# Dizzy-cell/HOUV

Measured on AMD Instinct MI355X. Metric: registration pairs/sec (2048-pt partial pairs), higher is better.
Workload: dtype f32; 1 GPU; HOUV solve_model, 2048x2048-pt pairs, batch 256/GPU, K=64 restarts x 200 Adam iterations + retry stages (BASELINE configs[1]); pairs_per_gpu=256, points=2048, kernel=64, iters=200, icp_refine=False, parallelism=dp1 (pair shards, one RCCL all-gather of [steps*P,12] per rank)

## Files before the change

houv_amd/_lib.py:

```python
import ctypes
import os

import torch

_HERE = os.path.dirname(os.path.abspath(__file__))
LIB_PATH = os.environ.get("HOUV_HIP_LIB") or os.path.join(_HERE, "lib", "libhouv_hip.so")
ABI_VERSION = 2

_c_f = ctypes.c_void_p
_int = ctypes.c_int
_dbl = ctypes.c_double
_flt = ctypes.c_float

_SIGNATURES = {
    "houv_abi_version": (ctypes.c_int, []),
    "houv_last_error": (ctypes.c_char_p, []),
    "houv_build_id": (ctypes.c_char_p, []),
    "houv_debug_set": (ctypes.c_int, [ctypes.c_char_p, ctypes.c_longlong]),
    "houv_chamfer_forward": (ctypes.c_int, [_c_f, _c_f, _int, _int, _int, _c_f, _c_f, _c_f, _c_f, _c_f]),
    "houv_chamfer_backward": (ctypes.c_int, [_c_f, _c_f, _int, _int, _int, _c_f, _c_f, _c_f, _c_f, _c_f, _c_f, _c_f]),
    "houv_kabsch": (ctypes.c_int, [_c_f, _c_f, _c_f, _int, _int, _c_f, _c_f, _c_f]),
    "houv_solve_iterate": (ctypes.c_int, [_c_f, _c_f, _int, _int, _int, _int, _c_f, _int, _int, _int, _int, _int, _int,
                                          _int, _int, _dbl, _dbl, _dbl, _dbl, _flt, _c_f, _c_f, _c_f, _c_f, _c_f, _c_f,
                                          _c_f]),
    "houv_solve_iterate_large": (ctypes.c_int, [_c_f, _c_f, _int, _int, _int, _int, _c_f, _int, _int, _int, _int, _int, _int,
                                                _int, _int, _dbl, _dbl, _dbl, _dbl, _flt, _c_f, _c_f, _c_f, _c_f, _c_f, _c_f,
                                                _c_f]),
    "houv_solve_iterate_pruned": (ctypes.c_int, [_c_f, _c_f, _int, _int, _int, _int, _c_f, _int, _int, _int, _int, _int,
                                                 _int, _int, _int, _dbl, _dbl, _dbl, _dbl, _flt, _c_f, _c_f, _c_f, _c_f,
                                                 _c_f, _c_f, _c_f, _int, _int, _c_f]),
    "houv_solve_variant": (ctypes.c_int, [_int, _int, _int, ctypes.POINTER(ctypes.c_int), ctypes.POINTER(ctypes.c_int),
                                          ctypes.POINTER(ctypes.c_int)]),
    "houv_solve_lds_bytes": (ctypes.c_longlong, [_int, _int, _int]),
    "houv_solve_walk_variant": (ctypes.c_int, [_int]),
    "houv_kd_sort": (ctypes.c_int, [_c_f, _int, _int, _int, _int, _c_f, _c_f, _c_f]),
    "houv_icp_refine": (ctypes.c_int, [_c_f, _c_f, _int, _int, _int, _c_f, _flt, _int, _flt, _flt, _c_f, _c_f, _c_f, _c_f, _c_f]),
    "houv_knn": (ctypes.c_int, [_c_f, _int, _int, _int, _c_f, _c_f]),
    "houv_edgeconv1": (ctypes.c_int, [_c_f, _c_f, _int, _int, _int, _c_f, _c_f, _c_f, _c_f, _c_f]),
    "houv_max_over_k": (ctypes.c_int, [_c_f, ctypes.c_longlong, _int, _int, _c_f, _int, _c_f]),
    "houv_gemm_f32": (ctypes.c_int, [_c_f, _c_f, _c_f, _int, _int, _int, _int, _int, _int, _int, _int, _int] +
                      [ctypes.c_longlong] * 6 + [_flt, _c_f, _c_f, _c_f, _int, ctypes.c_longlong, ctypes.c_longlong,
                                                 _int, _c_f]),
    "houv_attention_f32": (ctypes.c_int, [_c_f, _c_f, _c_f, _c_f, _int, _int, _int, _int, _int, _int, _int, _int, _int] +
                           [ctypes.c_longlong] * 4 + [_flt, _c_f]),
    "houv_layernorm": (ctypes.c_int, [_c_f, ctypes.c_longlong, _int, _c_f, _c_f, _flt, _c_f, _c_f, _c_f]),
    "houv_softmax_rows": (ctypes.c_int, [_c_f, ctypes.c_longlong, _int, _c_f]),
    "houv_softmax_corr": (ctypes.c_int, [_c_f, _int, _int, _int, _c_f, _c_f, _c_f]),
    "houv_furthest_point_sample": (ctypes.c_int, [_c_f, _int, _int, _int, _c_f, _c_f]),
    "houv_knn_cross": (ctypes.c_int, [_c_f, _c_f, _int, _int, _int, _int, _c_f, _c_f, _c_f]),
    "houv_gather_points": (ctypes.c_int, [_c_f, _c_f, _int, _int, _int, _int, _c_f, _c_f]),
    "houv_ball_query": (ctypes.c_int, [_c_f, _c_f, _int, _int, _int, _flt, _flt, _int, _c_f, _c_f, _c_f]),
    "houv_three_interpolate": (ctypes.c_int, [_c_f, _c_f, _c_f, _int, _int, _int, _int, _c_f, _c_f]),
    "houv_scatter_points_grad": (ctypes.c_int, [_c_f, _c_f, _c_f, _int, _int, _int, _int, _int, _c_f, _c_f, _c_f]),
    "houv_scatter_points_workspace_bytes": (ctypes.c_longlong, [_int, _int, _int]),
    "houv_emd_forward": (ctypes.c_int, [_c_f, _c_f, _int, _int, _int, _flt, _int, _c_f, _c_f, _c_f, _c_f, _c_f]),
    "houv_emd_workspace_bytes": (ctypes.c_longlong, [_int, _int]),
    "houv_emd_backward": (ctypes.c_int, [_c_f, _c_f, _int, _int, _c_f, _c_f, _c_f, _c_f]),
    "houv_rri_features": (ctypes.c_int, [_c_f, _c_f, _int, _int, _int, _int, _int, _c_f, _c_f]),
    "houv_gmm_params": (ctypes.c_int, [_c_f, _c_f, _int, _int, _int, _c_f, _c_f, _c_f, _c_f]),
    "houv_gmm_register": (ctypes.c_int, [_c_f, _c_f, _c_f, _c_f, _int, _int, _c_f, _c_f]),
    "houv_idam_simmat": (ctypes.c_int, [_c_f] * 4 + [_int] * 4 + [_c_f] * 15),
    "houv_edge_diff": (ctypes.c_int, [_c_f, _c_f, _int, _int, _int, _int, _int, _int, _c_f, _c_f]),
    "houv_mlp2_max": (ctypes.c_int, [_c_f, _int, _int, _int, _c_f, _int, _c_f, ctypes.c_longlong, _c_f, _c_f, _int, _c_f, _c_f, _c_f, _c_f]),
    "houv_mlp2_max_workspace_bytes": (ctypes.c_longlong, [_int, _int, _int]),
    "houv_mlp2_max_arg": (ctypes.c_int, [_c_f, _int, _int, _int, _c_f, _int, _c_f, ctypes.c_longlong, _c_f, _c_f, _int, _c_f, _c_f, _c_f, _c_f, _c_f]),
    "houv_mlp2_max_arg_workspace_bytes": (ctypes.c_longlong, [_int, _int, _int]),
    "houv_mlp2_max_backward": (ctypes.c_int, [_c_f, _int, _int, _int, _c_f, _int, _c_f, ctypes.c_longlong, _c_f, _int, _c_f, _c_f,
                                              _c_f, _c_f, _c_f, _int] + [_c_f] * 9),
    "houv_mlp2_max_backward_workspace_bytes": (ctypes.c_longlong, [_int] * 6),
    "houv_mlp2_max_backward_rows": (ctypes.c_int, [_int, _int, _int]),
    "houv_pcn_fold": (ctypes.c_int, [_c_f, _c_f, _c_f, _int, _int, _int, _c_f, _c_f, _c_f, _c_f, _c_f, _c_f, _c_f]),
    "houv_pcn_fold_backward": (ctypes.c_int, [_c_f, _c_f, _c_f, _int, _int, _int] + [_c_f] * 14 + [ctypes.c_longlong, _c_f]),
    "houv_pcn_fold_backward_workspace_bytes": (ctypes.c_longlong, [_int, _int, _int]),
    "houv_knn_feat": (ctypes.c_int, [_c_f, _int, _int, _int, _int, _int, _c_f, _c_f, _c_f]),
    "houv_dense_conv": (ctypes.c_int, [_c_f, _int, _c_f, _int, _int, _int, _int] + [_c_f] * 6 + [_int, _c_f, _int, _c_f]),
    "houv_dense_conv_arg": (ctypes.c_int, [_c_f, _int, _c_f, _int, _int, _int, _int] + [_c_f] * 6 + [_int, _c_f, _int, _c_f, _c_f]),
    "houv_dense_conv_backward": (ctypes.c_int, [_c_f, _int, _c_f, _int, _int, _int, _int] + [_c_f] * 6 +
                                 [_int, _c_f, _c_f, _int, _c_f, _int, _c_f, _int] + [_c_f] * 7 + [ctypes.c_longlong, _c_f]),
    "houv_dense_conv_backward_workspace_bytes": (ctypes.c_longlong, [_int, _int, _int, _int]),
    "houv_sa_attn": (ctypes.c_int, [_c_f, _int, _c_f, _int, _c_f, _int, _int, _int, _int] + [_c_f] * 5 + [_int, _c_f, _int, _c_f]),
    "houv_sa_attn_backward": (ctypes.c_int, [_c_f, _int, _c_f, _int, _int, _int, _int, _c_f, _c_f, _c_f, _c_f, _int, _c_f, _int, _c_f, _int,
                                             _c_f, _c_f, _c_f, _c_f, ctypes.c_longlong, _c_f]),
    "houv_sa_attn_backward_workspace_bytes": (ctypes.c_longlong, [_int, _int, _int, _int]),
    "houv_edge_pool": (ctypes.c_int, [_c_f, _int, _c_f, _c_f, _int, _int, _int, _int, _int, _c_f, _int, _c_f, _c_f]),
    "houv_edge_pool_backward": (ctypes.c_int, [_c_f, _int, _c_f, _c_f, _c_f, _int, _int, _int, _int, _int, _c_f, _int, _c_f,
                                               ctypes.c_longlong, _c_f]),
    "houv_edge_pool_backward_workspace_bytes": (ctypes.c_longlong, [_int, _int, _int, _int]),
    "houv_ef_expand": (ctypes.c_int, [_c_f, _int, _c_f, _int, _int, _int, _int, _int, _c_f, _int, _c_f, _c_f, _c_f, _int, _c_f, _c_f]),
    "houv_ef_expand_backward": (ctypes.c_int, [_c_f, _int, _c_f, _c_f, _int, _int, _int, _int, _int, _c_f, _int, _c_f, _c_f, _int, _c_f,
                                               _int, _c_f, _c_f, _c_f, _c_f, ctypes.c_longlong, _c_f]),
    "houv_ef_expand_backward_workspace_bytes": (ctypes.c_longlong, [_int] * 5),
    "houv_pose_forward": (ctypes.c_int,[_c_f, _int, _int, _int, _c_f, _int, _c_f, _c_f, _c_f, _c_f]),
}

_lib = None


class HouvHipError(RuntimeError):
    pass


def exported_symbols():
    return sorted(_SIGNATURES)


def load():
    global _lib
    if _lib is not None:
        return _lib
    if not os.path.exists(LIB_PATH):
        raise HouvHipError(
            f"{LIB_PATH} not found: build it with `python -c 'import __graft_entry__ as g; g.build()'` "
            "(or `make -C houv_amd/csrc`). houv_amd has no CPU fallback.")
    lib = ctypes.CDLL(LIB_PATH)
    for name, (res, args) in _SIGNATURES.items():
        fn = getattr(lib, name)
        fn.restype = res
        fn.argtypes = args
    if lib.houv_abi_version() != ABI_VERSION:
        raise HouvHipError(f"libhouv_hip.so ABI {lib.houv_abi_version()} != expected {ABI_VERSION}")
    _lib = lib
    return lib


def solve_variant(N, M, pruned=False, with_mode=False):
    b, q, m = ctypes.c_int(0), ctypes.c_int(0), ctypes.c_int(0)
    check(load().houv_solve_variant(int(N), int(M), int(bool(pruned)), ctypes.byref(b), ctypes.byref(q), ctypes.byref(m)),
          "houv_solve_variant")
    return (b.value, q.value, m.value) if with_mode else (b.value, q.value)


def solve_walk_variant(need):
    v = load().houv_solve_walk_variant(int(need))
    if v < 0:
        raise HouvHipError(f"houv_solve_walk_variant failed: {last_error()}")
    return v


def build_id():
    return load().houv_build_id().decode()


def debug_set(name, value):
    check(load().houv_debug_set(name.encode(), int(value)), "houv_debug_set")


def last_error():
    return load().houv_last_error().decode("utf-8", "replace")


def check(ok, what):
    if ok != 1:
        raise HouvHipError(f"{what} failed: {last_error()}")


def ptr(t):
    return None if t is None else ctypes.c_void_p(t.data_ptr())


def stream_of(t):
    return ctypes.c_void_p(torch.cuda.current_stream(t.device).cuda_stream)


def require_gpu(*tensors, dtype=None):
    for t in tensors:
        if t is None:
            continue
        if not t.is_cuda:
            raise HouvHipError("houv_amd ops run on an MI355X only: got a CPU tensor (there is no CPU fallback)")
        if not t.is_contiguous():
            raise HouvHipError("houv_amd ops need contiguous tensors")
    dev = [t.device for t in tensors if t is not None]
    if any(d != dev[0] for d in dev):
        raise HouvHipError("all tensors must live on the same device")


def require_gpu_any(*tensors):
    ts = [t for t in tensors if t is not None]
    for t in ts:
        if not t.is_cuda:
            raise HouvHipError("houv_amd ops run on an MI355X only: got a CPU tensor (there is no CPU fallback)")
        if t.dtype != torch.float32:
            raise HouvHipError(f"expected float32, got {t.dtype}")
    if any(t.device != ts[0].device for t in ts):
        raise HouvHipError("all tensors must live on the same device")
```

houv_amd/csrc/capi.hip:

```cpp
#include <stdarg.h>
#include <string.h>

#include "../../include/houv_hip.h"
#include "houv_common.h"

namespace houv {

static thread_local char g_err[512] = "";

void set_error(const char* fmt, ...) {
  va_list ap;
  va_start(ap, fmt);
  vsnprintf(g_err, sizeof(g_err), fmt, ap);
  va_end(ap);
  fprintf(stderr, "[houv_hip] %s\n", g_err);
}

DebugKnobs g_debug;

namespace {

__global__ void pose_kernel(const float* __restrict__ params, int n, int angle_base, int trans_mode,
                            float* __restrict__ R, float* __restrict__ T) {
  const int i = blockIdx.x * blockDim.x + threadIdx.x;
  if (i >= n) return;
  float p[8];
#pragma unroll
  for (int k = 0; k < 8; ++k) p[k] = params[i * 8 + k];
  Pose f;
  pose_forward(p, angle_base, trans_mode, f);
#pragma unroll
  for (int k = 0; k < 9; ++k) R[i * 9 + k] = f.R[k];
#pragma unroll
  for (int k = 0; k < 3; ++k) T[i * 3 + k] = f.T[k];
}

__global__ void move_kernel(const float* __restrict__ src, const float* __restrict__ R, const float* __restrict__ T,
                            size_t total, int N, float* __restrict__ moved) {
  for (size_t e = (size_t)blockIdx.x * blockDim.x + threadIdx.x; e < total; e += (size_t)gridDim.x * blockDim.x) {
    const size_t b = e / N;
    const float* r = R + b * 9;
    const float x = src[e * 3 + 0], y = src[e * 3 + 1], z = src[e * 3 + 2];
    moved[e * 3 + 0] = __builtin_fmaf(z, r[2], __builtin_fmaf(y, r[1], x * r[0])) + T[b * 3 + 0];
    moved[e * 3 + 1] = __builtin_fmaf(z, r[5], __builtin_fmaf(y, r[4], x * r[3])) + T[b * 3 + 1];
    moved[e * 3 + 2] = __builtin_fmaf(z, r[8], __builtin_fmaf(y, r[7], x * r[6])) + T[b * 3 + 2];
  }
}

}
}

extern "C" int houv_abi_version(void) { return HOUV_ABI_VERSION; }

extern "C" const char* houv_last_error(void) { return houv::g_err; }

extern "C" int houv_debug_set(const char* name, long long value) {
  using namespace houv;
  const struct { const char* name; std::atomic<int>* knob; long long lo, hi, step; } ints[] = {
      {"solve_predict", &g_debug.pred_mode, 0, 2, 1}, {"knn_split", &g_debug.knn_split, 0, 1, 1},
      {"attn_split", &g_debug.attn_split, 0, 1, 1},   {"gemm_split", &g_debug.gemm_split, 0, 6, 3}};
  if (name && !strcmp(name, "solve_stats")) {
    g_debug.stats = (unsigned long long)value;
    return 1;
  }
  if (name && !strcmp(name, "solve_walk_hist")) {
    g_debug.walk_hist = (unsigned long long)value;
    return 1;
  }
  if (name && !strcmp(name, "solve_cull_stats")) {
    g_debug.cull_stats = (unsigned long long)value;
    return 1;
  }
  for (const auto& k : ints)
    if (name && !strcmp(name, k.name) && value >= k.lo && value <= k.hi && value % k.step == 0) {
      *k.knob = (int)value;
      return 1;
    }
  set_error("houv_debug_set: unknown switch or value out of range: %s = %lld", name ? name : "(null)", value);
  return 0;
}

#ifndef HOUV_BUILD_ID
#define HOUV_BUILD_ID "unknown"
#endif
extern "C" const char* houv_build_id(void) { return HOUV_BUILD_ID; }

extern "C" int houv_pose_forward(const float* params, int n, int angle_base, int trans_mode, const float* src, int N,
                                 float* R, float* T, float* moved, void* stream) {
  using namespace houv;
  if (n < 0 || !params || !R || !T || angle_base < 0 || angle_base > 3 || trans_mode < 0 || trans_mode > 1) {
    set_error("houv_pose_forward: bad argument");
    return 0;
  }
  if (n == 0) return 1;
  hipStream_t s = (hipStream_t)stream;
  pose_kernel<<<(n + 255) / 256, 256, 0, s>>>(params, n, angle_base, trans_mode, R, T);
  if (src && moved && N > 0) {
    const size_t total = (size_t)n * N;
    size_t blocks = (total + 255) / 256;
    if (blocks > 16384) blocks = 16384;
    move_kernel<<<(unsigned)blocks, 256, 0, s>>>(src, R, T, total, N, moved);
  }
  return check_launch("houv_pose_forward") ? 1 : 0;
}
```

houv_amd/csrc/houv_common.h:

```cpp
#pragma once
#include <hip/hip_runtime.h>
#include <stdint.h>
#include <stdio.h>

#include <atomic>

#include "houv_math.h"

namespace houv {

constexpr int kWave = 64;
constexpr int kSub = 32;
constexpr int kTrk = 16;

void set_error(const char* fmt, ...);
struct SolveCommon;
__attribute__((visibility("hidden"))) int solve_check_args(const char* who, const SolveCommon& a, int use_views);
__attribute__((visibility("hidden"))) bool scatter_index_launch(const int* keys, int B, int N, int M, int* offsets, int* order,
                                                                hipStream_t stream);
inline bool check_launch(const char* what) {
  hipError_t e = hipGetLastError();
  if (e != hipSuccess) {
    set_error("%s: %s", what, hipGetErrorString(e));
    return false;
  }
  return true;
}

struct DebugKnobs {
  std::atomic<int> pred_mode{0};
  std::atomic<unsigned long long> stats{0ull};
  std::atomic<unsigned long long> walk_hist{0ull};
  std::atomic<unsigned long long> cull_stats{0ull};
  std::atomic<int> knn_split{1};
  std::atomic<int> attn_split{1};
  std::atomic<int> gemm_split{6};
};
extern DebugKnobs g_debug;

template <int MET>
__device__ __forceinline__ float metric_sqdist(float dx, float dy, float dz) {
  if constexpr (MET == 0) return __builtin_fmaf(dz, dz, __builtin_fmaf(dy, dy, dx * dx));
  else if constexpr (MET == 1) return __builtin_fmaf(dz, dz, dy * dy);
  else if constexpr (MET == 2) return __builtin_fmaf(dz, dz, dx * dx);
  else return __builtin_fmaf(dy, dy, dx * dx);
}

__device__ __forceinline__ float min3f(float a, float b, float c) {
  return __builtin_fminf(__builtin_fminf(a, b), c);
}

__device__ __forceinline__ float wave_sum(float v) {
#pragma unroll
  for (int o = 32; o > 0; o >>= 1) v += __shfl_xor(v, o, kWave);
  return v;
}

__device__ __forceinline__ int wave_sum_i(int v) {
#pragma unroll
  for (int o = 32; o > 0; o >>= 1) v += __shfl_xor(v, o, kWave);
  return v;
}

template <int CTRL, int ROW_MASK = 0xf, int BANK_MASK = 0xf>
__device__ __forceinline__ float dpp_f(float v) {
  return __int_as_float(__builtin_amdgcn_update_dpp(0, __float_as_int(v), CTRL, ROW_MASK, BANK_MASK, true));
}
template <int CTRL, int ROW_MASK = 0xf, int BANK_MASK = 0xf>
__device__ __forceinline__ int dpp_i(int v) {
  return __builtin_amdgcn_update_dpp(0, v, CTRL, ROW_MASK, BANK_MASK, true);
}

__device__ __forceinline__ float wave_sum_to_lane63(float v) {
  v += dpp_f<0x111>(v);
  v += dpp_f<0x112>(v);
  v += dpp_f<0x114>(v);
  v += dpp_f<0x118>(v);
  v += dpp_f<0x142, 0xa>(v);
  v += dpp_f<0x143, 0xc>(v);
  return v;
}

__device__ __forceinline__ int wave_max_to_lane63(int v) {
  v = max(v, dpp_i<0x111>(v));
  v = max(v, dpp_i<0x112>(v));
  v = max(v, dpp_i<0x114>(v));
  v = max(v, dpp_i<0x118>(v));
  v = max(v, dpp_i<0x142, 0xa>(v));
  v = max(v, dpp_i<0x143, 0xc>(v));
  return v;
}

template <int CTRL, int ROW_MASK = 0xf>
__device__ __forceinline__ float fmax_dpp(float v) {
  return __builtin_fmaxf(v, __int_as_float(__builtin_amdgcn_update_dpp(__float_as_int(v), __float_as_int(v), CTRL, ROW_MASK, 0xf, false)));
}
__device__ __forceinline__ float wave_fmax_to_lane63(float v) {
  v = fmax_dpp<0x111>(v);
  v = fmax_dpp<0x112>(v);
  v = fmax_dpp<0x114>(v);
  v = fmax_dpp<0x118>(v);
  v = fmax_dpp<0x142, 0xa>(v);
  v = fmax_dpp<0x143, 0xc>(v);
  return v;
}

__device__ __forceinline__ int wave_incl_scan_dpp(int x) {
  int v = x + dpp_i<0x111>(x);
  v += dpp_i<0x112>(x);
  v += dpp_i<0x113>(x);
  v += dpp_i<0x114, 0xf, 0xe>(v);
  v += dpp_i<0x118, 0xf, 0xc>(v);
  v += dpp_i<0x142, 0xa>(v);
  v += dpp_i<0x143, 0xc>(v);
  return v;
}

__device__ __forceinline__ int wave_incl_scan_i(int v) {
  const int lane = threadIdx.x & 63;
#pragma unroll
  for (int o = 1; o < 64; o <<= 1) {
    int n = __shfl_up(v, o, kWave);
    if (lane >= o) v += n;
  }
  return v;
}

}
```

houv_amd/csrc/houv_math.h:

```cpp
#pragma once
#include <math.h>

#if defined(__HIPCC__)
#define HOUV_HD __host__ __device__
#else
#define HOUV_HD
#endif

namespace houv {

constexpr float kPiF = 3.14159274101257324f;

enum TransMode { kTransHouv = 0, kTransSolve = 1 };

HOUV_HD inline float tsqrt(float x) { return sqrtf(x); }
HOUV_HD inline double tsqrt(double x) { return sqrt(x); }

struct Pose {
  float R[9];
  float T[3];
  float u[3], inv_vnorm, sin_t, cos_t, chat[3], inv_cnorm, sigma, a, s;
};

HOUV_HD inline void pose_forward(const float p[8], int angle_base, int trans_mode, Pose& o) {
// ... 90 lines not shown
  bool bad = false;
#pragma unroll
  for (int m = 0; m < 4; ++m) r.cd[m][0] = r.cd[m][1] = 0.f;
#pragma unroll
  for (int m = 0; m < NMET; ++m) {
    const float kk = (float)((m == 0) ? k_full : k_view);
    r.cd[m][0] = acc[(m * 2 + 0) * acc_stride] / kk;
    r.cd[m][1] = acc[(m * 2 + 1) * acc_stride] / kk;
    pick[m] = (r.cd[m][0] <= r.cd[m][1]) ? 0 : 1;
    val[m] = r.cd[m][pick[m]];
    if (r.cd[m][0] != r.cd[m][0] || r.cd[m][1] != r.cd[m][1]) { val[m] = NAN; bad = true; }
    const float w = ((m == 0) ? 6.0f : 1.0f) * loss_scale / kk;
    const float* ac = acc + (m * 2 + pick[m]) * acc_stride;
#pragma unroll
    for (int i = 0; i < 3; ++i) gT[i] += w * ac[1 + i];
#pragma unroll
    for (int i = 0; i < 9; ++i) Mm[i] += w * ac[4 + i];
  }
  r.score = val[0];
  r.loss = val[0] * 6.0f;
  if constexpr (NMET == 4) r.loss = r.loss + (val[1] + val[2] + val[3]);
  if (bad) {
#pragma unroll
    for (int i = 0; i < 3; ++i) gT[i] = NAN;
#pragma unroll
    for (int i = 0; i < 9; ++i) Mm[i] = NAN;
  }
  pose_backward(f, trans_mode, gT, Mm, r.g);
}

HOUV_HD inline void solve_tail_step(const float g[8], double* state, int f64_params, AdamScalars asc, double beta1, double beta2,
                                    double eps, int angle_base, int trans_mode, Pose& next) {
  if (f64_params) {
    for (int k = 0; k < 8; ++k)
      adam_step<double>(state[k], state[8 + k], state[16 + k], (double)g[k], asc, beta1, beta2, eps);
  } else {
    for (int k = 0; k < 8; ++k) {
      float pp = (float)state[k], mm = (float)state[8 + k], vv = (float)state[16 + k];
      adam_step<float>(pp, mm, vv, g[k], asc, beta1, beta2, eps);
      state[k] = pp; state[8 + k] = mm; state[16 + k] = vv;
    }
  }
  float p[8];
#pragma unroll
  for (int k = 0; k < 8; ++k) p[k] = (float)state[k];
  pose_forward(p, angle_base, trans_mode, next);
}

constexpr int kTermAnchorFloats = 20;
constexpr float kTermRel = 1e-3f;
constexpr float kTermAbs = 1e-6f;
constexpr float kTermMoveErr = 1e-6f;

template <int NMET>
HOUV_HD inline unsigned term_masks(const float* anchor, const float* R, const float* T, float radius) {
  float fr = 0.f, ft = 0.f, tn = 0.f, ta = 0.f;
#pragma unroll
  for (int i = 0; i < 9; ++i) {
    const float d = R[i] - anchor[8 + i];
    fr += d * d;
  }
#pragma unroll
  for (int i = 0; i < 3; ++i) {
    const float d = T[i] - anchor[17 + i];
    ft += d * d;
    tn += T[i] * T[i];
    ta += anchor[17 + i] * anchor[17 + i];
  }
  const float delta2 = 2.0f * (sqrtf(fr) * radius + sqrtf(ft));
  const float abs_margin = kTermAbs + kTermMoveErr * (2.0f * radius + sqrtf(tn) + sqrtf(ta));
  unsigned need = ((1u << NMET) - 1u) * 0x11u;
#pragma unroll
  for (int m = 0; m < NMET; ++m) {
    const float c0 = anchor[2 * m], c1 = anchor[2 * m + 1];
    const float slack = delta2 + kTermRel * (fabsf(c0) + fabsf(c1) + delta2) + abs_margin;
    const unsigned drop1 = (c0 + slack < c1) ? (0x10u << m) : 0u;
    const unsigned drop0 = (c1 + slack < c0) ? (1u << m) : 0u;
    need &= ~(drop0 | drop1);
  }
  return need;
}

constexpr float kTermDefectMax = 1e-3f;
constexpr float kTermDefectErr = 1e-6f;

HOUV_HD inline float term_rot_defect(const float* M) {
  float s = 0.f;
#pragma unroll
  for (int i = 0; i < 3; ++i)
#pragma unroll
    for (int j = i; j < 3; ++j) {
      const float g = M[i] * M[j] + M[3 + i] * M[3 + j] + M[6 + i] * M[6 + j] - ((i == j) ? 1.0f : 0.0f);
      s += ((i == j) ? 1.0f : 2.0f) * g * g;
    }
  return sqrtf(s) + kTermDefectErr;
}

HOUV_HD inline void term_travel(const float* Rz, const float* Tz, const float* R, const float* T, float def_now, float radius,
                                float& d, float& tz) {
  float fr = 0.f, ft = 0.f, ta = 0.f;
#pragma unroll
  for (int i = 0; i < 9; ++i) {
    const float e = R[i] - Rz[i];
    fr += e * e;
  }
#pragma unroll
  for (int i = 0; i < 3; ++i) {
    const float e = T[i] - Tz[i];
    ft += e * e;
    ta += Tz[i] * Tz[i];
  }
  const float fro = sqrtf(fr), defect = def_now + term_rot_defect(Rz);
  const float tight = fro * 0.70710683f + 2.0f * defect;
  const bool ok = (fr <= 2.0f) & (defect <= kTermDefectMax) & (tight < fro);
  d = (ok ? tight : fro) * radius + sqrtf(ft);
  tz = sqrtf(ta);
}

template <int NMET>
HOUV_HD inline unsigned term_anchor_masks(const float* cd, const float* fresh, const float* stale, int stride,
                                          unsigned stale_bits, const float* R, const float* T, float radius_in) {
  const float radius = fabsf(radius_in);
  const float def_now = term_rot_defect(R);
  const float tn = sqrtf(T[0] * T[0] + T[1] * T[1] + T[2] * T[2]);
  float d_f, t_f;
  term_travel(fresh, fresh + 9, R, T, def_now, radius, d_f, t_f);
  unsigned need = ((1u << NMET) - 1u) * 0x11u;
#pragma unroll
  for (int m = 0; m < NMET; ++m) {
    float Rs[9], Ts[3], d_s, t_s;
#pragma unroll
    for (int i = 0; i < 9; ++i) Rs[i] = stale[(m * 12 + i) * stride];
#pragma unroll
    for (int i = 0; i < 3; ++i) Ts[i] = stale[(m * 12 + 9 + i) * stride];
    term_travel(Rs, Ts, R, T, def_now, radius, d_s, t_s);
    const bool s0 = (stale_bits >> m) & 1u, s1 = (stale_bits >> (4 + m)) & 1u;
    const float d0 = s0 ? d_s : d_f, d1 = s1 ? d_s : d_f;
    const float t0 = s0 ? t_s : t_f, t1 = s1 ? t_s : t_f;
    const float c0 = cd[2 * m], c1 = cd[2 * m + 1];
    const float dd = d0 + d1;
    const float slack = dd + kTermRel * (fabsf(c0) + fabsf(c1) + dd) + kTermAbs +
                        kTermMoveErr * (2.0f * radius + tn + 0.5f * (t0 + t1));
    const unsigned drop1 = (c0 + slack < c1) ? (0x10u << m) : 0u;
    const unsigned drop0 = (c1 + slack < c0) ? (1u << m) : 0u;
    need &= ~(drop0 | drop1);
  }
  return need;
}

constexpr int kWalkSets[] = {6, 11, 12, 13, 15};
constexpr int kNumWalkSets = (int)(sizeof(kWalkSets) / sizeof(kWalkSets[0]));
constexpr int walk_step_cost(unsigned mset) {
  const int k0 = (int)(mset & 1u), k1 = (int)((mset >> 1) & 1u), k2 = (int)((mset >> 2) & 1u), k3 = (int)((mset >> 3) & 1u);
  return 16 * (2 * (k0 + k1 + k2 + ((k0 | k3) ? 1 : 0)) + 2 * k1 + (k0 + k1 + k2 + k3)) + 5 * (k0 + k1 + k2 + k3);
}
constexpr bool walk_instantiated(unsigned mset) {
  for (int i = 0; i < kNumWalkSets; ++i)
    if ((unsigned)kWalkSets[i] == mset) return true;
  return false;
}
constexpr unsigned walk_variant(unsigned need) {
  unsigned best = 15u;
  for (int i = 0; i < kNumWalkSets; ++i) {
    const unsigned s = (unsigned)kWalkSets[i];
    if ((s & need) == need && walk_step_cost(s) < walk_step_cost(best)) best = s;
  }
  return best;
}
static_assert(walk_instantiated(15u) && walk_variant(15u) == 15u && walk_step_cost(15u) == 16 * 14 + 20, "today's code is a variant");
constexpr unsigned long long walk_variant_table() {
  unsigned long long t = 0ull;
  for (unsigned n = 0; n < 16u; ++n) t |= (unsigned long long)walk_variant(n) << (4 * n);
  return t;
}

HOUV_HD inline float box_med3(float a, float b, float c) {
#if defined(__HIP_DEVICE_COMPILE__)
  return __builtin_amdgcn_fmed3f(a, b, c);
#else
  if (a != a || b != b || c != c) return fminf(fminf(a, b), c);
  return fmaxf(fminf(a, b), fminf(fmaxf(a, b), c));
#endif
}

template <int NMET>
HOUV_HD inline bool box_within_bounds(float dx, float dy, float dz, const float* b, unsigned mset) {
  if constexpr (NMET == 4) {
    const float xx = dx * dx, yy = dy * dy;
    const float s3 = __builtin_fmaf(dy, dy, xx), s1 = __builtin_fmaf(dz, dz, yy), s2 = __builtin_fmaf(dz, dz, xx);
    const float s0 = __builtin_fmaf(dz, dz, s3);
    bool in = false;
    if (mset & 1u) in |= s0 <= b[0];
    if (mset & 2u) in |= s1 <= b[1];
    if (mset & 4u) in |= s2 <= b[2];
    if (mset & 8u) in |= s3 <= b[3];
    return in;
  } else {
    return __builtin_fmaf(dz, dz, __builtin_fmaf(dy, dy, dx * dx)) <= b[0];
  }
}

template <int NMET>
HOUV_HD inline bool box_test_query(const float* q, const float* lo, const float* hi, const float* ub, unsigned mset) {
  return box_within_bounds<NMET>(q[0] - box_med3(q[0], lo[0], hi[0]), q[1] - box_med3(q[1], lo[1], hi[1]),
                                 q[2] - box_med3(q[2], lo[2], hi[2]), ub, mset);
}

HOUV_HD inline float box_group_gap(float glo, float ghi, float lo, float hi) {
  return fmaxf(fmaxf(fminf(lo, hi) - ghi, glo - fmaxf(lo, hi)), 0.0f);
}

template <int NMET>
HOUV_HD inline bool box_test_group(const float* glo, const float* ghi, const float* lo, const float* hi, const float* gub,
                                   unsigned mset) {
  return box_within_bounds<NMET>(box_group_gap(glo[0], ghi[0], lo[0], hi[0]), box_group_gap(glo[1], ghi[1], lo[1], hi[1]),
                                 box_group_gap(glo[2], ghi[2], lo[2], hi[2]), gub, mset);
}

template <typename T>
HOUV_HD inline void svd3x3(const T H[9], T U[9], T S[3], T V[9]) {
  T B[9];
  for (int i = 0; i < 9; ++i) { B[i] = H[i]; V[i] = (i % 4 == 0) ? (T)1 : (T)0; }
  const int P[3] = {0, 0, 1}, Qi[3] = {1, 2, 2};
  for (int sweep = 0; sweep < 12; ++sweep) {
    T off = 0;
    for (int r = 0; r < 3; ++r) {
      const int p = P[r], q = Qi[r];
      const T a = B[0 * 3 + p] * B[0 * 3 + p] + B[1 * 3 + p] * B[1 * 3 + p] + B[2 * 3 + p] * B[2 * 3 + p];
      const T b = B[0 * 3 + q] * B[0 * 3 + q] + B[1 * 3 + q] * B[1 * 3 + q] + B[2 * 3 + q] * B[2 * 3 + q];
      const T g = B[0 * 3 + p] * B[0 * 3 + q] + B[1 * 3 + p] * B[1 * 3 + q] + B[2 * 3 + p] * B[2 * 3 + q];
      const T eps2 = sizeof(T) == 4 ? (T)1e-14 : (T)1e-31;
      if (g * g <= eps2 * a * b) continue;
      off += (T)1;
      const T zeta = (b - a) / ((T)2 * g);
      const T az = zeta < 0 ? -zeta : zeta;
      const T t = (zeta < 0 ? (T)-1 : (T)1) / (az + tsqrt((T)1 + zeta * zeta));
      const T c = (T)1 / tsqrt((T)1 + t * t);
      const T s = c * t;
      for (int i = 0; i < 3; ++i) {
        const T bp = B[i * 3 + p], bq = B[i * 3 + q];
        B[i * 3 + p] = c * bp - s * bq;
        B[i * 3 + q] = s * bp + c * bq;
        const T vp = V[i * 3 + p], vq = V[i * 3 + q];
        V[i * 3 + p] = c * vp - s * vq;
        V[i * 3 + q] = s * vp + c * vq;
      }
    }
    if (off == (T)0) break;
  }
  for (int j = 0; j < 3; ++j)
    S[j] = tsqrt(B[0 * 3 + j] * B[0 * 3 + j] + B[1 * 3 + j] * B[1 * 3 + j] + B[2 * 3 + j] * B[2 * 3 + j]);
  auto swapcol = [&](int x, int y) {
    T ts = S[x]; S[x] = S[y]; S[y] = ts;
    for (int i = 0; i < 3; ++i) {
      T tb = B[i * 3 + x]; B[i * 3 + x] = B[i * 3 + y]; B[i * 3 + y] = tb;
      T tv = V[i * 3 + x]; V[i * 3 + x] = V[i * 3 + y]; V[i * 3 + y] = tv;
    }
  };
  if (S[0] < S[1]) swapcol(0, 1);
  if (S[1] < S[2]) swapcol(1, 2);
  if (S[0] < S[1]) swapcol(0, 1);
  const T tiny = S[0] * (sizeof(T) == 4 ? (T)1e-6 : (T)1e-13);
  for (int j = 0; j < 2; ++j) {
    if (S[j] > tiny && S[j] > (T)0) {
      for (int i = 0; i < 3; ++i) U[i * 3 + j] = B[i * 3 + j] / S[j];
    } else if (j == 0) {
      U[0] = 1; U[3] = 0; U[6] = 0;
    } else {
      const T x = U[0], y = U[3], z = U[6];
      const T ax = x < 0 ? -x : x, ay = y < 0 ? -y : y, az = z < 0 ? -z : z;
      T e[3] = {0, 0, 0};
      if (ax <= ay && ax <= az) e[0] = 1; else if (ay <= az) e[1] = 1; else e[2] = 1;
      T w[3] = {y * e[2] - z * e[1], z * e[0] - x * e[2], x * e[1] - y * e[0]};
      const T n = tsqrt(w[0] * w[0] + w[1] * w[1] + w[2] * w[2]);
      U[1] = w[0] / n; U[4] = w[1] / n; U[7] = w[2] / n;
    }
  }
  if (S[2] > tiny && S[2] > (T)0) {
    for (int i = 0; i < 3; ++i) U[i * 3 + 2] = B[i * 3 + 2] / S[2];
  } else {
    U[2] = U[3] * U[7] - U[6] * U[4];
    U[5] = U[6] * U[1] - U[0] * U[7];
    U[8] = U[0] * U[4] - U[3] * U[1];
  }
}

template <typename T>
HOUV_HD inline T det3(const T m[9]) {
  return m[0] * (m[4] * m[8] - m[5] * m[7]) - m[1] * (m[3] * m[8] - m[5] * m[6]) + m[2] * (m[3] * m[7] - m[4] * m[6]);
}

template <typename T>
HOUV_HD inline void kabsch_rotation(const T H[9], T R[9]) {
  T U[9], S[3], V[9];
  svd3x3<T>(H, U, S, V);
  for (int i = 0; i < 3; ++i)
    for (int j = 0; j < 3; ++j) R[i * 3 + j] = V[i * 3 + 0] * U[j * 3 + 0] + V[i * 3 + 1] * U[j * 3 + 1] + V[i * 3 + 2] * U[j * 3 + 2];
  if (det3<T>(R) < (T)0) {
    for (int i = 0; i < 3; ++i)
      for (int j = 0; j < 3; ++j) R[i * 3 + j] = V[i * 3 + 0] * U[j * 3 + 0] + V[i * 3 + 1] * U[j * 3 + 1] - V[i * 3 + 2] * U[j * 3 + 2];
  }
}

}
```

houv_amd/csrc/solve.hip:

```cpp
#include <stddef.h>
#include <stdlib.h>

#include "../../include/houv_hip.h"
#include "houv_common.h"
#include "houv_solve.h"

namespace houv {
namespace {

struct SolveArgs : SolveCommon {
  short* nn_ws;
  int ws_valid;
  int ws_stride;
  int pred_mode;
  unsigned long long* stats;
  unsigned long long* walk_hist;
  unsigned long long* cull_stats;
};

constexpr int kRescanBatch = 4;
constexpr int kRefresh = 4;
constexpr int kTermMaxAge = 0;

struct Smem {
  float4* tgt;
  float4* mov;
  double* state;
  double* adam;
  float* pose;
  float* acc;
  float* red;
  unsigned* hist;
  int* ctl;
  float4* tbox;
  float4* mbox;
  SortedStage st;
  float* anchor;
};
constexpr int kAnchorFloats = kTermAnchorFloats + 4;
constexpr int kTermAges = 8;
constexpr int kStalePose = 4;


__host__ __device__ inline int pad_unit(int prune) { return prune == 3 ? 2 * kSub : kSub; }

__host__ __device__ inline size_t smem_bytes(int N, int M, int block, int prune, int q) {
  const int pu = pad_unit(prune);
  int npad = (N + pu - 1) / pu * pu, mpad = (M + pu - 1) / pu * pu;
  if (prune) npad = mpad = (npad > mpad ? npad : mpad);
  const int nw = block / 64;
  const size_t nq = (size_t)block * q;
  return (size_t)(npad + mpad) * 16 + 28 * 8 + kPoseFloats * 4 + 8 * kAccStride * 4 + (size_t)2 * nw * kRedStride * 4 +
         kHistSets * kHistBins * 4 + (8 + nw) * 4 + 64 + (prune ? 2 * 128 * 16 + nq * 2 + 132 * 4 + kAnchorFloats * 4 : 0);
}

__device__ inline Smem carve(unsigned char* base, int N, int M, int block, int nq, int pu) {
  int npad = (N + pu - 1) / pu * pu, mpad = (M + pu - 1) / pu * pu;
  if (nq) npad = mpad = (npad > mpad ? npad : mpad);
  const int nw = block / 64;
  Smem s;
  s.tgt = reinterpret_cast<float4*>(base);
  s.mov = s.tgt + mpad;
  s.state = reinterpret_cast<double*>(s.mov + npad);
  s.adam = s.state + 24;
  s.pose = reinterpret_cast<float*>(s.adam + 4);
  s.acc = s.pose + kPoseFloats;
  s.red = s.acc + 8 * kAccStride;
  s.hist = reinterpret_cast<unsigned*>(s.red + 2 * nw * kRedStride);
  s.ctl = reinterpret_cast<int*>(s.hist + kHistSets * kHistBins);
  const size_t box_off = ((size_t)(reinterpret_cast<unsigned char*>(s.ctl + 8 + nw) - base) + 15) & ~(size_t)15;
  s.tbox = reinterpret_cast<float4*>(base + box_off);
  s.mbox = s.tbox + 128;
  s.st.hist = reinterpret_cast<int*>(s.mbox + 128);
  s.st.order = reinterpret_cast<unsigned short*>(s.st.hist + 132);
  s.anchor = reinterpret_cast<float*>(s.st.order + nq);
  return s;
}

template <typename T>
__device__ __forceinline__ T fresh(T v) {
  asm volatile("" : "+s"(v));
  return v;
}
__device__ __forceinline__ const float* fresh_lds(const float* p) {
  typedef const float __attribute__((address_space(3))) * lds_f;
  return (const float*)(lds_f)(size_t)fresh((unsigned)(size_t)(lds_f)p);
}

template <int BLOCK, int Q>
__device__ __forceinline__ void select_smallest(const unsigned (&key)[Q], int ksel, unsigned* hist, int* ctl,
                                                bool (&sel)[Q], int& hrot) {
  constexpr int NW = BLOCK / 64;
  const int tid = tid_x(), lane = tid & 63, wave = tid >> 6;
  RadixState rs{0u, 0u, ksel, 0};
#pragma unroll
  for (int pass = 0; pass < 4; ++pass) {
    unsigned* h = radix_rotate<BLOCK>(hist, hrot, tid);
#pragma unroll
    for (int k = 0; k < Q; ++k) radix_count(h, key[k], pass, lane, rs);
    __syncthreads();
    radix_pick(h, pass, lane, rs);
  }
  const unsigned prefix = rs.prefix;
  const int remaining = rs.remaining, neq = rs.neq;
  if (neq == remaining) {
#pragma unroll
    for (int k = 0; k < Q; ++k) sel[k] = key[k] <= prefix;
  } else {
    int e = 0;
#pragma unroll
    for (int k = 0; k < Q; ++k) e += (key[k] == prefix) ? 1 : 0;
    const int incl = wave_incl_scan_dpp(e);
    __syncthreads();
    if (lane == 63) ctl[8 + wave] = incl;
    __syncthreads();
    int rank = incl - e;
    for (int w = 0; w < NW; ++w) rank += (w < wave) ? ctl[8 + w] : 0;
#pragma unroll
    for (int k = 0; k < Q; ++k) {
      const bool eq = key[k] == prefix;
      sel[k] = key[k] < prefix || (eq && rank < remaining);
      rank += eq ? 1 : 0;
    }
  }
}

constexpr int kGradN = 12;

__device__ __forceinline__ void park(float v, float* dst) {
  v = wave_sum_to_lane63(v);
  if ((tid_x() & 63) == 63) *dst = v;
}

template <int BLOCK, int Q, int NMET>
__device__ __forceinline__ void select_all(const Smem& sm, const float (&best)[Q][NMET], int count, int k_full, int k_view,
                                           unsigned need, int& hrot, unsigned (&bits)[NMET]) {
  bool valid[Q], sel[Q];
  unsigned key[Q];
#pragma unroll
  for (int m = 0; m < NMET; ++m) {
    const int ksel = (m == 0) ? k_full : k_view;
#pragma unroll
    for (int k = 0; k < Q; ++k) {
      valid[k] = pt_index<BLOCK>(k) < count;
      key[k] = valid[k] ? __float_as_uint(best[k][m]) : 0xFFFFFFFFu;
      sel[k] = valid[k];
    }
    if (ksel < count && ((need >> m) & 1u)) select_smallest<BLOCK, Q>(key, ksel, sm.hist, sm.ctl, sel, hrot);
    unsigned b = 0u;
#pragma unroll
    for (int k = 0; k < Q; ++k) b |= sel[k] ? (1u << k) : 0u;
    bits[m] = b;
  }
}

template <int Q>
__device__ __forceinline__ float lane_sqrt_sum(const float (&bd)[Q], unsigned selbits) {
  float s = 0.f;
#pragma unroll
  for (int k = 0; k < Q; ++k)
    if ((selbits >> k) & 1u) s += (bd[k] < INFINITY) ? sqrtf(bd[k]) : NAN;
  return s;
}

template <int BLOCK, int Q, int MET, int DIR, bool WS>
__device__ __forceinline__ void lane_grad_sums(const Smem& sm, const float4* __restrict__ refs, const float (&qx)[Q],
                                               const float (&qy)[Q], const float (&qz)[Q], const float (&bd)[Q],
                                               const int (&bt)[Q], unsigned selbits, int count, const float (&px)[Q],
                                               const float (&py)[Q], const float (&pz)[Q], float (&g)[kGradN], buf_t ws,
                                               int ws_off) {
  const int rot = tid_x() & (kSub - 1);
#pragma unroll
  for (int i = 0; i < kGradN; ++i) g[i] = 0.f;
  float R[9], T[3];
  if constexpr (DIR == 0) load_rt(sm.pose, R, T);
#pragma unroll
  for (int k = 0; k < Q; ++k) {
    int jn;
    const float4 nn = recover_nn<MET, kRescanBatch, true>(refs + bt[k] * kTrk, qx[k], qy[k], qz[k], bd[k], rot, jn);
    if (WS && pt_index<BLOCK>(k) < count)
      __builtin_amdgcn_raw_buffer_store_b16((unsigned short)(bt[k] * kTrk + jn), ws, tid_x() * kNnRec,
                                            ws_off + pt_base<BLOCK>(k) * kNnRec + MET * 2, 0);
    if ((selbits >> k) & 1u) {
      const float s = (bd[k] < INFINITY) ? sqrtf(bd[k]) : NAN;
      const float inv = 1.0f / s;
      float dx, dy, dz, sx, sy, sz;
      if constexpr (DIR == 1) {
        dx = qx[k] - nn.x; dy = qy[k] - nn.y; dz = qz[k] - nn.z;
        sx = px[k]; sy = py[k]; sz = pz[k];
      } else {
        dx = nn.x - qx[k]; dy = nn.y - qy[k]; dz = nn.z - qz[k];
        const float ux = nn.x - T[0], uy = nn.y - T[1], uz = nn.z - T[2];
        sx = R[0] * ux + R[3] * uy + R[6] * uz;
        sy = R[1] * ux + R[4] * uy + R[7] * uz;
        sz = R[2] * ux + R[5] * uy + R[8] * uz;
      }
      if constexpr (MET == 1) dx = 0.f;
      if constexpr (MET == 2) dy = 0.f;
      if constexpr (MET == 3) dz = 0.f;
      const float cx = dx * inv, cy = dy * inv, cz = dz * inv;
      g[0] += cx; g[1] += cy; g[2] += cz;
      g[3] += cx * sx; g[4] += cx * sy; g[5] += cx * sz;
      g[6] += cy * sx; g[7] += cy * sy; g[8] += cy * sz;
      g[9] += cz * sx; g[10] += cz * sy; g[11] += cz * sz;
    }
  }
}

template <int BLOCK, int Q, int NMET>
__device__ __forceinline__ void park_sqrt_sums(const float (&best)[Q][NMET], const unsigned (&selbits)[NMET], unsigned need,
                                               float* red_wave) {
  float bd[Q];
#pragma unroll
  for (int m = 0; m < NMET; ++m) {
    if (!((need >> m) & 1u)) continue;
#pragma unroll
    for (int k = 0; k < Q; ++k) bd[k] = best[k][m];
    park(lane_sqrt_sum<Q>(bd, selbits[m]), red_wave + m * kAccN);
  }
}

template <int BLOCK, int Q, int NMET, int DIR, bool WS>
__device__ __forceinline__ void park_grad_sums(const Smem& sm, const float4* __restrict__ refs, const float (&qx)[Q],
                                               const float (&qy)[Q], const float (&qz)[Q], const float (&best)[Q][NMET],
                                               const int (&btile)[Q][NMET], const unsigned (&selbits)[NMET], unsigned mask,
                                               int count, const float (&px)[Q], const float (&py)[Q], const float (&pz)[Q],
                                               float* red_wave, buf_t ws, int ws_off) {
  float bd[Q], g[kGradN];
  int bt[Q];
#define HOUV_GRAD(MET)                                                                                              \
  if ((mask >> MET) & 1u) {                                                                                         \
    _Pragma("unroll") for (int k = 0; k < Q; ++k) {                                                                 \
      bd[k] = best[k][MET];                                                                                         \
      bt[k] = btile[k][MET];                                                                                        \
    }                                                                                                               \
    lane_grad_sums<BLOCK, Q, MET, DIR, WS>(sm, refs, qx, qy, qz, bd, bt, selbits[MET], count, px, py, pz, g,        \
                                           ws, ws_off);                                                             \
    _Pragma("unroll") for (int i = 0; i < kGradN; ++i) park(g[i], red_wave + MET * kAccN + 1 + i);                  \
  }
  HOUV_GRAD(0)
  if constexpr (NMET == 4) {
    HOUV_GRAD(1)
    HOUV_GRAD(2)
    HOUV_GRAD(3)
  }
#undef HOUV_GRAD
}

template <int BLOCK, int NMET>
__device__ __forceinline__ void final_sums(const Smem& sm, int dir, bool want_s, unsigned grad_mask, unsigned need) {
  constexpr int NW = BLOCK / 64;
  const int tid = tid_x();
  if (tid < NMET * kAccN) {
    const int m = tid / kAccN, i = tid % kAccN;
    if ((i == 0) ? want_s : (((grad_mask >> m) & 1u) != 0u)) {
      const float* r = sm.red + (size_t)dir * NW * kRedStride + tid;
      float a = 0.f;
#pragma unroll
      for (int w = 0; w < NW; ++w) a += r[w * kRedStride];
      if (i == 0 && !((need >> m) & 1u)) a = INFINITY;
      sm.acc[(m * 2 + dir) * kAccStride + i] = a;
    }
  }
}

template <int NMET>
__device__ __forceinline__ unsigned picked_direction(const Smem& sm, int k_full, int k_view) {
  unsigned pick = 0u;
#pragma unroll
  for (int m = 0; m < NMET; ++m) {
    const float kk = (float)((m == 0) ? k_full : k_view);
    const float cd0 = sm.acc[(m * 2 + 0) * kAccStride] / kk, cd1 = sm.acc[(m * 2 + 1) * kAccStride] / kk;
    pick |= (cd0 <= cd1) ? 0u : (1u << m);
  }
  return pick;
}

template <int BLOCK>
__device__ __forceinline__ void load_src_point(buf_t src, int k, int N, float& x, float& y, float& z) {
  x = y = z = 0.f;
  if (pt_index<BLOCK>(k) < N) {
    const auto v = __builtin_amdgcn_raw_buffer_load_b96(src, tid_x() * 12, pt_base<BLOCK>(k) * 12, 0);
    x = __uint_as_float(v[0]); y = __uint_as_float(v[1]); z = __uint_as_float(v[2]);
  }
}

template <int BLOCK, int Q, int MET>
__device__ __forceinline__ void repair_direction_a(const Smem& sm, buf_t src, int N, int mpad, int k_sel,
                                                   int& hrot, float* red_wave) {
  float sx[Q], sy[Q], sz[Q], mx[Q], my[Q], mz[Q];
  float R[9], T[3];
  load_rt(sm.pose, R, T);
#pragma unroll
  for (int k = 0; k < Q; ++k) {
    load_src_point<BLOCK>(src, k, N, sx[k], sy[k], sz[k]);
    move_point(R, T, sx[k], sy[k], sz[k], mx[k], my[k], mz[k]);
  }
  float bd[Q];
  int bt[Q];
  sweep_one<Q, MET>(sm.tgt, mpad / kTrk, mx, my, mz, bd, bt);
  bool sel[Q];
  unsigned key[Q], bits = 0u;
#pragma unroll
  for (int k = 0; k < Q; ++k) {
    sel[k] = pt_index<BLOCK>(k) < N;
    key[k] = sel[k] ? __float_as_uint(bd[k]) : 0xFFFFFFFFu;
  }
  if (k_sel < N) select_smallest<BLOCK, Q>(key, k_sel, sm.hist, sm.ctl, sel, hrot);
#pragma unroll
  for (int k = 0; k < Q; ++k) bits |= sel[k] ? (1u << k) : 0u;
  float g[kGradN];
  lane_grad_sums<BLOCK, Q, MET, 1, false>(sm, sm.tgt, mx, my, mz, bd, bt, bits, N, sx, sy, sz, g, src, 0);
#pragma unroll
  for (int i = 0; i < kGradN; ++i) park(g[i], red_wave + MET * kAccN + 1 + i);
}

template <int BLOCK, int Q, int NMET, int PRUNE>
__global__ __launch_bounds__(BLOCK, (Q == 1 ? 8 : 4)) void solve_kernel(SolveArgs a) {
  static_assert(PRUNE == 0 || PRUNE == 2 || PRUNE == 3, "brute force, or the balanced walk over sub-tiles / super-tiles");
  constexpr int TS = (PRUNE == 3) ? 1 : 0;
  constexpr int kPad = kSub << TS;
  extern __shared__ __attribute__((aligned(512))) unsigned char smem_raw[];
  const int N = a.N, M = a.M;
  const Smem sm = carve(smem_raw, N, M, BLOCK, PRUNE ? BLOCK * Q : 0, kPad);
  const int tid = tid_x();
  const int ninst = a.P * a.K;
  int inst = blockIdx.x;
  if ((ninst & 7) == 0) inst = (blockIdx.x & 7) * (ninst >> 3) + (blockIdx.x >> 3);
  const int pair = inst / a.K;
  const buf_t src = make_buf(a.src + (size_t)pair * N * 3, N * 12);
  const float* __restrict__ tgt = a.tgt + (size_t)pair * M * 3;
  const int npad = (N + kPad - 1) / kPad * kPad, mpad = (M + kPad - 1) / kPad * kPad;
  const float4 pad4 = make_float4(INFINITY, INFINITY, INFINITY, 0.f);

  for (int j = tid; j < mpad; j += BLOCK) sm.tgt[j] = (j < M) ? make_float4(tgt[j * 3], tgt[j * 3 + 1], tgt[j * 3 + 2], 0.f) : pad4;
  for (int j = N + tid; j < npad; j += BLOCK) sm.mov[j] = pad4;
  if (tid < 24) sm.state[tid] = a.state[(size_t)inst * 24 + tid];
  for (int j = tid; j < kHistBins; j += BLOCK) sm.hist[j] = 0u;
  if constexpr (PRUNE) {
    if (tid < 132) sm.st.hist[tid] = 0;
  }
  int hrot = 0;
  __syncthreads();
  buf_t ws = src;
  const int ws_b = 0, ws_a = a.ws_stride * kNnRec;
  float4* ws_res = nullptr;
  if constexpr (PRUNE) {
    ws = make_buf(a.nn_ws + (size_t)inst * 16 * a.ws_stride, 32 * a.ws_stride);
    ws_res = reinterpret_cast<float4*>(a.nn_ws + ((size_t)inst * 16 + 8) * a.ws_stride);
    float tx0[Q], ty0[Q], tz0[Q];
#pragma unroll
    for (int k = 0; k < Q; ++k) {
      const int i = pt_index<BLOCK>(k);
      const float4 v = (i < M) ? sm.tgt[i] : make_float4(0.f, 0.f, 0.f, 0.f);
      tx0[k] = v.x; ty0[k] = v.y; tz0[k] = v.z;
    }
    tile_boxes<BLOCK, Q, TS>(tx0, ty0, tz0, M, mpad / kPad, sm.tbox);
  }
  constexpr int kAdamTid = BLOCK >= 128 ? 64 : 0;
  if (tid == 0) {
    float p[8];
#pragma unroll
    for (int k = 0; k < 8; ++k) p[k] = (float)sm.state[k];
    Pose f;
    pose_forward(p, a.angle_base, a.trans_mode, f);
    store_pose(sm.pose, f);
  }
  if (tid == kAdamTid) {
    const int step = a.steps_done + 1;
    const AdamScalars asc = adam_scalars(step, a.lr, a.beta1, a.beta2);
    sm.adam[(step & 1) * 2 + 0] = asc.step_size;
    sm.adam[(step & 1) * 2 + 1] = asc.bc2_sqrt;
  }
  if constexpr (PRUNE) {
    float r2 = 0.f;
#pragma unroll
    for (int k = 0; k < Q; ++k) {
      float x, y, z;
      load_src_point<BLOCK>(src, k, N, x, y, z);
      const float v = __builtin_fmaf(z, z, __builtin_fmaf(y, y, x * x));
      r2 = (v <= r2) ? r2 : ((v < INFINITY) ? v : INFINITY);
    }
#pragma unroll
    for (int o = 1; o < 64; o <<= 1) r2 = fmaxf(r2, __shfl_xor(r2, o, 64));
    if ((tid & 63) == 0) sm.red[tid >> 6] = r2;
    if (tid == 0) {
      sm.ctl[0] = (int)(((1u << NMET) - 1u) * 0x11u);
      reinterpret_cast<unsigned*>(sm.anchor)[kTermAges] = 0u;
    }
  }
  __syncthreads();
  if constexpr (PRUNE) {
    if (tid == 0) {
      float r2 = 0.f;
      for (int w = 0; w < BLOCK / 64; ++w) r2 = fmaxf(r2, sm.red[w]);
      sm.anchor[kTermAnchorFloats] = sqrtf(r2) * 1.000001f;
    }
  }

  unsigned long long clk0 = 0ull, rt0 = 0ull;
  if (a.stats) {
    clk0 = __builtin_amdgcn_s_memtime();
    rt0 = __builtin_amdgcn_s_memrealtime();
  }
  constexpr int NW = BLOCK / 64;
  constexpr unsigned kAllMet = (1u << NMET) - 1u;
  unsigned pred_a = kAllMet;
  auto red_row = [&](int dir) { return sm.red + ((size_t)dir * NW + (tid_x() >> 6)) * kRedStride; };
#pragma unroll 1
  for (int it = 0; it < a.n_iters; ++it) {
    if (a.pred_mode == 1) pred_a = 0u;
    const bool allgrad = a.pred_mode == 2 || ((PRUNE != 0) && (((a.steps_done + it) % kRefresh) == 0 || (a.ws_valid == 0 && it == 0)));
    unsigned need_a = kAllMet, need_b = kAllMet;
    if constexpr (PRUNE != 0) {
      const unsigned w = (unsigned)__builtin_amdgcn_readfirstlane(*reinterpret_cast<const int*>(fresh_lds(reinterpret_cast<const float*>(sm.ctl))));
      need_b = w & kAllMet;
      need_a = (w >> 4) & kAllMet;
    }
    const unsigned grad_a = (allgrad ? kAllMet : (pred_a | ~need_b)) & need_a;
    {
      float sx[Q], sy[Q], sz[Q], mx[Q], my[Q], mz[Q];
      float R[9], T[3];
      load_rt(fresh_lds(sm.pose), R, T);
#pragma unroll
      for (int k = 0; k < Q; ++k) {
        const int i = pt_index<BLOCK>(k);
        const bool ok = i < N;
        load_src_point<BLOCK>(src, k, N, sx[k], sy[k], sz[k]);
        move_point(R, T, sx[k], sy[k], sz[k], mx[k], my[k], mz[k]);
        if (ok) sm.mov[i] = make_float4(mx[k], my[k], mz[k], 0.f);
      }
      __syncthreads();
      bool pruned_now = false;
      float best[Q][NMET];
      int btile[Q][NMET];
      if constexpr (PRUNE) {
        tile_boxes<BLOCK, Q, TS>(mx, my, mz, N, npad / kPad, sm.mbox);
        pruned_now = (a.ws_valid != 0) || (it > 0);
      }
      if (need_a != 0u) {
        if (pruned_now) {
          if constexpr (PRUNE != 0)
            pruned_sweep_sorted<BLOCK, Q, NMET, TS>(sm.tgt, sm.tbox, mpad / kPad, sm.mbox, sm.mov, sm.tgt, sm.mov, mx, my, mz, ws, ws_a, N,
                                                need_a, sm.st, ws_res, best, btile, a.stats, fresh(a.walk_hist), fresh(a.cull_stats));
        } else {
          sweep<Q, NMET>(sm.tgt, mpad / kTrk, mx, my, mz, best, btile);
          if (a.stats && (tid & 63) == 0) atomicAdd(&a.stats[3], 1ull);
        }
        unsigned sel[NMET];
        select_all<BLOCK, Q, NMET>(sm, best, N, a.k_full, a.k_view, need_a, hrot, sel);
        park_sqrt_sums<BLOCK, Q, NMET>(best, sel, need_a, red_row(1));
        park_grad_sums<BLOCK, Q, NMET, 1, PRUNE != 0>(sm, sm.tgt, mx, my, mz, best, btile, sel, grad_a, N, sx, sy, sz, red_row(1), ws,
                                                     ws_a);
      }
      __syncthreads();
      final_sums<BLOCK, NMET>(sm, 1, true, grad_a, need_a);
    }
    unsigned pick_a;
    {
      float tx[Q], ty[Q], tz[Q];
#pragma unroll
      for (int k = 0; k < Q; ++k) {
        const int i = pt_index<BLOCK>(k);
        const float4 v = (i < M) ? sm.tgt[i] : make_float4(0.f, 0.f, 0.f, 0.f);
        tx[k] = v.x; ty[k] = v.y; tz[k] = v.z;
      }
      const bool pruned_now = (PRUNE != 0) && ((a.ws_valid != 0) || (it > 0));
      auto pick_winners = [&]() {
        __syncthreads();
        final_sums<BLOCK, NMET>(sm, 0, true, 0u, need_b);
        __syncthreads();
        pick_a = picked_direction<NMET>(sm, fresh(a.k_full), fresh(a.k_view));
        return (allgrad ? kAllMet : (~pick_a & kAllMet)) & need_b;
      };
      unsigned grad_b = 0u;
      if (need_b != 0u) {
        float best[Q][NMET];
        int btile[Q][NMET];
        if (pruned_now) {
          if constexpr (PRUNE != 0)
            pruned_sweep_sorted<BLOCK, Q, NMET, TS>(sm.mov, sm.mbox, npad / kPad, sm.tbox, sm.tgt, sm.tgt, sm.mov, tx, ty, tz, ws, ws_b, M,
                                                need_b, sm.st, ws_res, best, btile, a.stats, fresh(a.walk_hist), fresh(a.cull_stats));
        } else {
          sweep<Q, NMET>(sm.mov, npad / kTrk, tx, ty, tz, best, btile);
          if (a.stats && (tid & 63) == 0) atomicAdd(&a.stats[3], 1ull);
        }
        unsigned sel[NMET];
        select_all<BLOCK, Q, NMET>(sm, best, M, a.k_full, a.k_view, need_b, hrot, sel);
        park_sqrt_sums<BLOCK, Q, NMET>(best, sel, need_b, red_row(0));
        grad_b = pick_winners();
        park_grad_sums<BLOCK, Q, NMET, 0, PRUNE != 0>(sm, sm.mov, tx, ty, tz, best, btile, sel, grad_b, M, tx, ty, tz, red_row(0), ws,
                                                     ws_b);
      } else {
        pick_winners();
      }
      const unsigned miss = pick_a & ~grad_a & kAllMet;
      if (miss) {
        if (miss & 1u) repair_direction_a<BLOCK, Q, 0>(sm, src, N, mpad, a.k_full, hrot, red_row(1));
        if constexpr (NMET == 4) {
          if (miss & 2u) repair_direction_a<BLOCK, Q, 1>(sm, src, N, mpad, a.k_view, hrot, red_row(1));
          if (miss & 4u) repair_direction_a<BLOCK, Q, 2>(sm, src, N, mpad, a.k_view, hrot, red_row(1));
          if (miss & 8u) repair_direction_a<BLOCK, Q, 3>(sm, src, N, mpad, a.k_view, hrot, red_row(1));
        }
      }
      __syncthreads();
      final_sums<BLOCK, NMET>(sm, 0, false, grad_b, kAllMet);
      if (miss) final_sums<BLOCK, NMET>(sm, 1, false, miss, kAllMet);
    }
    pred_a = pick_a;
    static_assert(NMET * kAccN <= 64, "final_sums runs on the scalar tail's wave");
    __builtin_amdgcn_wave_barrier();

    if (kAdamTid != 0 && tid == kAdamTid && it + 1 < a.n_iters) {
      const int step = a.steps_done + it + 2;
      const AdamScalars asc = adam_scalars(step, fresh(a.lr), fresh(a.beta1), fresh(a.beta2));
      sm.adam[(step & 1) * 2 + 0] = asc.step_size;
      sm.adam[(step & 1) * 2 + 1] = asc.bc2_sqrt;
    }
    if (tid == 0) {
      const int k_full = fresh(a.k_full), k_view = fresh(a.k_view);
      const float loss_scale = fresh(a.loss_scale);
      const double lr = fresh(a.lr), beta1 = fresh(a.beta1), beta2 = fresh(a.beta2), eps = fresh(a.eps);
      const int angle_base = fresh(a.angle_base), trans_mode = fresh(a.trans_mode);
      Pose f;
      load_pose(f, sm.pose);
      TailLoss r;
      solve_tail_loss<NMET>(sm.acc, kAccStride, f, k_full, k_view, loss_scale, trans_mode, r);
      if (it == a.n_iters - 1)
        store_outputs(a.out_score, a.out_loss, a.out_R, a.out_T, a.out_grad, a.out_cd, inst, f, r);
      if constexpr (PRUNE != 0) {
#pragma unroll
        for (int m = 0; m < NMET; ++m) {
          if ((need_b >> m) & 1u) sm.anchor[2 * m] = r.cd[m][0];
          if ((need_a >> m) & 1u) sm.anchor[2 * m + 1] = r.cd[m][1];
        }
      }
      const int step = a.steps_done + it + 1;
      const AdamScalars asc{sm.adam[(step & 1) * 2 + 0], sm.adam[(step & 1) * 2 + 1]};
      solve_tail_step(r.g, sm.state, a.f64_params, asc, beta1, beta2, eps, angle_base, trans_mode, f);
      if constexpr (PRUNE != 0) {
        unsigned next = kAllMet | (kAllMet << 4), ages = 0u;
        const bool all_next = fresh(a.pred_mode) == 2 || it + 2 >= a.n_iters;
        if (!all_next) {
          const unsigned have = need_b | (need_a << 4);
          float* stale = reinterpret_cast<float*>(sm.tbox) + 3;
          next = term_anchor_masks<NMET>(sm.anchor, sm.pose, stale, kStalePose, ~have & 0xffu, f.R, f.T,
                                         sm.anchor[kTermAnchorFloats]);
          const unsigned old_ages = reinterpret_cast<const unsigned*>(sm.anchor)[kTermAges];
#pragma unroll
          for (int m = 0; m < NMET; ++m) {
            unsigned age = (old_ages >> (8 * m)) & 0xffu;
            age = (((next >> m) & (next >> (4 + m)) & 1u) != 0u) ? 0u : age + 1u;
            if (kTermMaxAge > 0 && age > (unsigned)kTermMaxAge) {
              next |= 0x11u << m;
              age = 0u;
            }
            if (age > 0xffu) age = 0xffu;
            ages |= age << (8 * m);
            if (((have & ~next) >> m) & 0x11u) {
#pragma unroll
              for (int i = 0; i < 12; ++i) stale[(m * 12 + i) * kStalePose] = sm.pose[i];
            }
          }
        }
        reinterpret_cast<unsigned*>(sm.anchor)[kTermAges] = ages;
        sm.ctl[0] = (int)next;
        if (a.stats) {
          atomicAdd(&a.stats[6], (unsigned long long)(__popc(need_a) + __popc(need_b)));
          atomicAdd(&a.stats[7], (unsigned long long)(2 * NMET));
        }
      }
      store_pose(sm.pose, f);
      if (kAdamTid == 0 && it + 1 < a.n_iters) {
        const AdamScalars nxt = adam_scalars(step + 1, lr, beta1, beta2);
        sm.adam[((step + 1) & 1) * 2 + 0] = nxt.step_size;
        sm.adam[((step + 1) & 1) * 2 + 1] = nxt.bc2_sqrt;
      }
    }
    __syncthreads();
  }
  if (tid_x() < 24) a.state[(size_t)inst * 24 + tid_x()] = sm.state[tid_x()];
  if (a.stats) {
    const unsigned long long dc = __builtin_amdgcn_s_memtime() - clk0, dr = __builtin_amdgcn_s_memrealtime() - rt0;
    if (tid == 0) {
      atomicAdd(&a.stats[4], dc);
      atomicAdd(&a.stats[5], dr);
    }
  }
}

template <int BLOCK, int Q, int PRUNE>
int launch(const SolveArgs& a, int use_views, hipStream_t s) {
  const size_t bytes = smem_bytes(a.N, a.M, BLOCK, PRUNE, Q);
  const int grid = a.P * a.K;
  hipError_t e;
  if (use_views) {
    e = hipFuncSetAttribute((const void*)solve_kernel<BLOCK, Q, 4, PRUNE>, hipFuncAttributeMaxDynamicSharedMemorySize, (int)bytes);
    if (e != hipSuccess) { set_error("houv_solve_iterate: cannot reserve %zu B of LDS: %s", bytes, hipGetErrorString(e)); return 0; }
    solve_kernel<BLOCK, Q, 4, PRUNE><<<grid, BLOCK, bytes, s>>>(a);
  } else {
    e = hipFuncSetAttribute((const void*)solve_kernel<BLOCK, Q, 1, PRUNE>, hipFuncAttributeMaxDynamicSharedMemorySize, (int)bytes);
    if (e != hipSuccess) { set_error("houv_solve_iterate: cannot reserve %zu B of LDS: %s", bytes, hipGetErrorString(e)); return 0; }
    solve_kernel<BLOCK, Q, 1, PRUNE><<<grid, BLOCK, bytes, s>>>(a);
  }
  return check_launch("houv_solve_iterate") ? 1 : 0;
}

}
}

extern "C" int houv_solve_variant(int N, int M, int pruned, int* block, int* points_per_lane, int* prune_mode) {
  using namespace houv;
  const int mx = N > M ? N : M;
  if (N <= 0 || M <= 0) {
    set_error("houv_solve_variant: bad cloud sizes N=%d M=%d", N, M);
    return 0;
  }
  if (mx > 4096) {
    set_error("houv_solve_iterate: clouds larger than 4096 points do not fit in 160 KiB of LDS (N=%d M=%d)", N, M);
    return 0;
  }
  int b, q;
  if (mx <= 64) { b = 64; q = 1; }
  else if (mx <= 128) { b = 128; q = 1; }
  else if (mx <= 256) { b = 256; q = 1; }
  else if (mx <= 512) { b = 256; q = 2; }
  else if (mx <= 768) { b = 256; q = 3; }
  else if (mx <= 1024) { b = 256; q = 4; }
  else if (mx <= 1536) { b = 512; q = 3; }
  else if (mx <= 2048) { b = 512; q = 4; }
  else if (mx <= 3072) { b = 1024; q = 3; }
  else { b = 1024; q = 4; }
  if (block) *block = b;
  if (points_per_lane) *points_per_lane = q;
  constexpr int kPrunedMinPoints = 257;
  if (prune_mode) *prune_mode = (!pruned || mx < kPrunedMinPoints) ? 0 : (mx > 2048) ? 3 : 2;
  return 1;
}

extern "C" int houv_solve_walk_variant(int need) {
  if (need < 0 || need > 15) {
    houv::set_error("houv_solve_walk_variant: the term mask of a direction is 0..15, got %d", need);
    return -1;
  }
  return (int)houv::walk_variant((unsigned)need);
}

extern "C" long long houv_solve_lds_bytes(int N, int M, int pruned) {
  using namespace houv;
  int block = 0, q = 0, mode = 0;
  if (!houv_solve_variant(N, M, pruned, &block, &q, &mode)) return -1;
  return (long long)smem_bytes(N, M, block, mode, q);
}

int houv::solve_check_args(const char* who, const SolveCommon& a, int use_views) {
  const int P = a.P, N = a.N, M = a.M;
  if (P < 0 || N <= 0 || M <= 0 || a.K <= 0 || a.n_iters <= 0 || a.steps_done < 0 || a.angle_base < 0 || a.angle_base > 3 ||
      a.trans_mode < 0 || a.trans_mode > 1) {
    set_error("%s: bad argument P=%d N=%d M=%d K=%d n_iters=%d steps_done=%d base=%d trans_mode=%d", who, P, N, M, a.K,
              a.n_iters, a.steps_done, a.angle_base, a.trans_mode);
    return 0;
  }
  if (P == 0) return 1;
  if (!a.src || !a.tgt || !a.state) {
    set_error("%s: null pointer", who);
    return 0;
  }
  const int kv = use_views ? a.k_view : 1;
  if (a.k_full < 1 || a.k_full > N || a.k_full > M || kv < 1 || kv > N || kv > M) {
    set_error("%s: top-k size out of range (k_full=%d k_view=%d N=%d M=%d)", who, a.k_full, a.k_view, N, M);
    return 0;
  }
  if ((long long)P * a.K > 0x7fffffffLL) {
    set_error("%s: too many hypotheses", who);
    return 0;
  }
  return 2;
}

static int solve_dispatch(const houv::SolveCommon& c, int use_views, short* nn_ws, int ws_valid, int ws_stride, bool prune,
                          void* stream, const char* who) {
  using namespace houv;
  const int ok = solve_check_args(who, c, use_views);
  if (ok < 2) return ok;
  const int N = c.N, M = c.M;
  SolveArgs a{c, nn_ws, ws_valid, ws_stride, g_debug.pred_mode.load(),
              reinterpret_cast<unsigned long long*>(g_debug.stats.load()),
              reinterpret_cast<unsigned long long*>(g_debug.walk_hist.load()),
              reinterpret_cast<unsigned long long*>(g_debug.cull_stats.load())};
  hipStream_t s = (hipStream_t)stream;
  const int mx = N > M ? N : M;
  int block = 0, q = 0, mode = 0;
  if (!houv_solve_variant(N, M, prune ? 1 : 0, &block, &q, &mode)) return 0;
  if (prune && (!nn_ws || ws_stride < mx || (ws_stride & 7))) {
    set_error("%s: pruned mode needs a workspace of 16 x ws_stride int16 per hypothesis, ws_stride >= max(N,M) and a multiple of 8", who);
    return 0;
  }
  if (prune && ((uintptr_t)nn_ws & 15)) {
    set_error("%s: the pruned-mode workspace must be 16-byte aligned", who);
    return 0;
  }
  if (prune && ws_valid < 0) {
    a.ws_valid = 0;
    mode = 0;
  }
  if (mode == 0) a.nn_ws = nullptr;
#define HOUV_GO(B_, Q_)                                                          \
  if (block == B_ && q == Q_) {                                                  \
    if (mode == 2) return launch<B_, Q_, ((B_ >= 256 && Q_ >= 2) ? 2 : 0)>(a, use_views, s);    \
    return launch<B_, Q_, 0>(a, use_views, s);                                   \
  }
  if (mx <= 2048) {
    HOUV_GO(64, 1) HOUV_GO(128, 1) HOUV_GO(256, 1) HOUV_GO(256, 2) HOUV_GO(256, 3) HOUV_GO(256, 4)
    HOUV_GO(512, 3) HOUV_GO(512, 4)
  } else {
    if (block == 1024 && q == 3) return mode == 3 ? launch<1024, 3, 3>(a, use_views, s) : launch<1024, 3, 0>(a, use_views, s);
    if (block == 1024 && q == 4) return mode == 3 ? launch<1024, 4, 3>(a, use_views, s) : launch<1024, 4, 0>(a, use_views, s);
  }
#undef HOUV_GO
  set_error("%s: no kernel variant <%d,%d>", who, block, q);
  return 0;
}

extern "C" int houv_solve_iterate(const float* src, const float* tgt, int P, int N, int M, int K, double* state,
                                  int steps_done, int n_iters, int angle_base, int trans_mode, int use_views,
                                  int f64_params, int k_full, int k_view, double lr, double beta1, double beta2,
                                  double eps, float loss_scale, float* out_score, float* out_loss, float* out_R,
                                  float* out_T, float* out_grad, float* out_cd, void* stream) {
  const houv::SolveCommon a{src, tgt, P, N, M, K, state, steps_done, n_iters, angle_base, trans_mode, f64_params, k_full, k_view,
                            lr, beta1, beta2, eps, loss_scale, out_score, out_loss, out_R, out_T, out_grad, out_cd};
  return solve_dispatch(a, use_views, nullptr, 0, 0, false, stream, "houv_solve_iterate");
}

extern "C" int houv_solve_iterate_pruned(const float* src, const float* tgt, int P, int N, int M, int K, double* state,
                                         int steps_done, int n_iters, int angle_base, int trans_mode, int use_views,
                                         int f64_params, int k_full, int k_view, double lr, double beta1, double beta2,
                                         double eps, float loss_scale, float* out_score, float* out_loss, float* out_R,
                                         float* out_T, float* out_grad, float* out_cd, int16_t* nn_ws, int ws_valid,
                                         int ws_stride, void* stream) {
  const houv::SolveCommon a{src, tgt, P, N, M, K, state, steps_done, n_iters, angle_base, trans_mode, f64_params, k_full, k_view,
                            lr, beta1, beta2, eps, loss_scale, out_score, out_loss, out_R, out_T, out_grad, out_cd};
  return solve_dispatch(a, use_views, (short*)nn_ws, ws_valid, ws_stride, true, stream, "houv_solve_iterate_pruned");
}
```

houv_amd/ops.py:

```python
import torch

from . import _lib

_F32, _I32, _F64 = torch.float32, torch.int32, torch.float64


def _want(t, dtype, name):
    if t.dtype != dtype:
        raise _lib.HouvHipError(f"{name}: expected {dtype}, got {t.dtype}")


def chamfer_forward(xyz1, xyz2, dist1, dist2, idx1, idx2):
    _lib.require_gpu(xyz1, xyz2, dist1, dist2, idx1, idx2)
    for t, d, n in ((xyz1, _F32, "xyz1"), (xyz2, _F32, "xyz2"), (dist1, _F32, "dist1"), (dist2, _F32, "dist2"),
                    (idx1, _I32, "idx1"), (idx2, _I32, "idx2")):
        _want(t, d, n)
    B, N, _ = xyz1.shape
    M = xyz2.shape[1]
    if xyz1.shape[2] != 3 or xyz2.shape[2] != 3 or xyz2.shape[0] != B:
        raise _lib.HouvHipError("chamfer_forward: expected xyz1[B,N,3], xyz2[B,M,3]")
    if dist1.numel() != B * N or idx1.numel() != B * N or dist2.numel() != B * M or idx2.numel() != B * M:
        raise _lib.HouvHipError("chamfer_forward: output shapes do not match [B,N] / [B,M]")
    with torch.cuda.device(xyz1.device):
        ok = _lib.load().houv_chamfer_forward(_lib.ptr(xyz1), _lib.ptr(xyz2), B, N, M, _lib.ptr(dist1), _lib.ptr(dist2),
                                              _lib.ptr(idx1), _lib.ptr(idx2), _lib.stream_of(xyz1))
    _lib.check(ok, "houv_chamfer_forward")
    return 1


def chamfer_backward(xyz1, xyz2, gradxyz1, gradxyz2, graddist1, graddist2, idx1, idx2):
    _lib.require_gpu(xyz1, xyz2, gradxyz1, gradxyz2, graddist1, graddist2, idx1, idx2)
    for t, d, n in ((xyz1, _F32, "xyz1"), (xyz2, _F32, "xyz2"), (gradxyz1, _F32, "gradxyz1"),
                    (gradxyz2, _F32, "gradxyz2"), (graddist1, _F32, "graddist1"), (graddist2, _F32, "graddist2"),
                    (idx1, _I32, "idx1"), (idx2, _I32, "idx2")):
        _want(t, d, n)
    B, N, _ = xyz1.shape
    M = xyz2.shape[1]
    if (gradxyz1.shape != xyz1.shape or gradxyz2.shape != xyz2.shape or graddist1.numel() != B * N
            or graddist2.numel() != B * M or idx1.numel() != B * N or idx2.numel() != B * M):
        raise _lib.HouvHipError("chamfer_backward: shape mismatch")
    with torch.cuda.device(xyz1.device):
        ok = _lib.load().houv_chamfer_backward(_lib.ptr(xyz1), _lib.ptr(xyz2), B, N, M, _lib.ptr(graddist1),
                                               _lib.ptr(graddist2), _lib.ptr(idx1), _lib.ptr(idx2), _lib.ptr(gradxyz1),
                                               _lib.ptr(gradxyz2), _lib.stream_of(xyz1))
    _lib.check(ok, "houv_chamfer_backward")
    return 1


def kabsch(src, corr, weights=None):
    _lib.require_gpu(src, corr, weights)
    _want(src, _F32, "src"); _want(corr, _F32, "corr")
    B, C, N = src.shape
    if C != 3 or corr.shape != src.shape:
        raise _lib.HouvHipError("kabsch: expected src, corr [B,3,N]")
    if weights is not None:
        _want(weights, _F32, "weights")
        if weights.numel() != B * N:
            raise _lib.HouvHipError("kabsch: expected weights [B,1,N]")
    R = torch.empty((B, 3, 3), dtype=_F32, device=src.device)
    t = torch.empty((B, 3), dtype=_F32, device=src.device)
    with torch.cuda.device(src.device):
        ok = _lib.load().houv_kabsch(_lib.ptr(src), _lib.ptr(corr), _lib.ptr(weights), B, N, _lib.ptr(R), _lib.ptr(t),
                                     _lib.stream_of(src))
    _lib.check(ok, "houv_kabsch")
    return R, t


def pose_forward(params, angle_base, trans_mode=0, src=None):
    _lib.require_gpu(params, src)
    _want(params, _F32, "params")
    n = params.shape[0]
    R = torch.empty((n, 3, 3), dtype=_F32, device=params.device)
    T = torch.empty((n, 3), dtype=_F32, device=params.device)
    moved, N = None, 0
    if src is not None:
        _want(src, _F32, "src")
        N = src.shape[1]
        moved = torch.empty_like(src)
    with torch.cuda.device(params.device):
        ok = _lib.load().houv_pose_forward(_lib.ptr(params), n, int(angle_base), int(trans_mode), _lib.ptr(src), N,
                                           _lib.ptr(R), _lib.ptr(T), _lib.ptr(moved), _lib.stream_of(params))
    _lib.check(ok, "houv_pose_forward")
    return (R, T) if src is None else (R, T, moved)


def solve_iterate_out(src, tgt, state, K, steps_done, n_iters, angle_base, trans_mode, use_views, f64_params, k_full,
                      k_view, lr, beta1, beta2, eps, loss_scale, out_score, out_loss, out_R, out_T, out_grad=None,
                      out_cd=None, nn_ws=None, ws_valid=0, large=False):
    _lib.require_gpu(src, tgt, state, out_score, out_loss, out_R, out_T, out_grad, out_cd, nn_ws)
    _want(src, _F32, "src"); _want(tgt, _F32, "tgt"); _want(state, _F64, "state")
    P, N, _ = src.shape
    M = tgt.shape[1]
    if tgt.shape[0] != P or src.shape[2] != 3 or tgt.shape[2] != 3:
        raise _lib.HouvHipError("solve_iterate: expected src[P,N,3], tgt[P,M,3]")
    n = P * int(K)
    if tuple(state.shape) != (n, 24):
        raise _lib.HouvHipError(f"solve_iterate: state must be [{n},24], got {tuple(state.shape)}")
    for t, numel, name in ((out_score, n, "out_score"), (out_loss, n, "out_loss"), (out_R, 9 * n, "out_R"),
                           (out_T, 3 * n, "out_T"), (out_grad, 8 * n, "out_grad"), (out_cd, 8 * n, "out_cd")):
        if t is not None:
            _want(t, _F32, name)
            if t.numel() != numel:
                raise _lib.HouvHipError(f"solve_iterate: {name} must hold {numel} floats, got {t.numel()}")
    common = (_lib.ptr(src), _lib.ptr(tgt), P, N, M, int(K), _lib.ptr(state), int(steps_done), int(n_iters),
              int(angle_base), int(trans_mode), int(bool(use_views)), int(bool(f64_params)), int(k_full), int(k_view),
              float(lr), float(beta1), float(beta2), float(eps), float(loss_scale), _lib.ptr(out_score),
              _lib.ptr(out_loss), _lib.ptr(out_R), _lib.ptr(out_T), _lib.ptr(out_grad), _lib.ptr(out_cd))
    if large and nn_ws is not None:
        raise _lib.HouvHipError("solve_iterate: the large-cloud kernel is a brute-force sweep and takes no workspace")
    with torch.cuda.device(src.device):
        if large:
            ok = _lib.load().houv_solve_iterate_large(*common, _lib.stream_of(src))
        elif nn_ws is None:
            ok = _lib.load().houv_solve_iterate(*common, _lib.stream_of(src))
        else:
            if nn_ws.dtype != torch.int16 or nn_ws.dim() != 3 or tuple(nn_ws.shape[:2]) != (n, 16) or not nn_ws.is_contiguous():
                raise _lib.HouvHipError("solve_iterate: nn_ws must be a contiguous int16 [P*K,16,stride] tensor (ops.solve_workspace)")
            ok = _lib.load().houv_solve_iterate_pruned(*common, _lib.ptr(nn_ws), int(ws_valid), nn_ws.shape[2],
                                                       _lib.stream_of(src))
    _lib.check(ok, "houv_solve_iterate" + ("_large" if large else "_pruned" if nn_ws is not None else ""))
    return 1


def solve_iterate_large_out(src, tgt, state, K, steps_done, n_iters, angle_base, trans_mode, use_views, f64_params, k_full,
                            k_view, lr, beta1, beta2, eps, loss_scale, out_score, out_loss, out_R, out_T, out_grad=None,
                            out_cd=None):
    return solve_iterate_out(src, tgt, state, K, steps_done, n_iters, angle_base, trans_mode, use_views, f64_params, k_full,
                             k_view, lr, beta1, beta2, eps, loss_scale, out_score, out_loss, out_R, out_T, out_grad, out_cd,
                             large=True)


def solve_workspace(n_hypotheses, N, M, device):
    stride = (max(int(N), int(M)) + 7) // 8 * 8
    return torch.empty((int(n_hypotheses), 16, stride), dtype=torch.int16, device=device)


def solve_iterate(src, tgt, state, K, *, steps_done, n_iters, angle_base, trans_mode, use_views, f64_params, k_full,
                  k_view, lr, loss_scale, betas=(0.9, 0.999), eps=1e-8, want_grad=False, want_cd=False, nn_ws=None,
                  ws_valid=False, large=False):
    _lib.require_gpu(src, tgt, state)
    dev = src.device
    n = src.shape[0] * int(K)
    out = dict(score=torch.empty(n, dtype=_F32, device=dev), loss=torch.empty(n, dtype=_F32, device=dev),
               R=torch.empty((n, 3, 3), dtype=_F32, device=dev), T=torch.empty((n, 3), dtype=_F32, device=dev))
    if want_grad:
        out["grad"] = torch.empty((n, 8), dtype=_F32, device=dev)
    if want_cd:
        out["cd"] = torch.empty((n, 8), dtype=_F32, device=dev)
    solve_iterate_out(src, tgt, state, K, steps_done, n_iters, angle_base, trans_mode, use_views, f64_params, k_full,
                      k_view, lr, betas[0], betas[1], eps, loss_scale, out["score"], out["loss"], out["R"], out["T"],
                      out.get("grad"), out.get("cd"), nn_ws, -1 if ws_valid == "verify" else int(bool(ws_valid)), large=large)
    return out


KD_RULES = {"area": 0, "extent": 1}


def kd_sort(cloud, leaf=32, rule="area", return_order=False):
    _lib.require_gpu(cloud)
    _want(cloud, _F32, "cloud")
    if cloud.dim() != 3 or cloud.shape[2] != 3:
        raise _lib.HouvHipError("kd_sort: expected cloud[P,N,3]")
    if rule not in KD_RULES:
        raise _lib.HouvHipError(f"kd_sort: rule must be one of {sorted(KD_RULES)}, got {rule!r}")
    P, N, _ = cloud.shape
    out = torch.empty_like(cloud)
    order = torch.empty((P, N), dtype=_I32, device=cloud.device) if return_order else None
    with torch.cuda.device(cloud.device):
        ok = _lib.load().houv_kd_sort(_lib.ptr(cloud), P, N, int(leaf), KD_RULES[rule], _lib.ptr(out), _lib.ptr(order),
                                      _lib.stream_of(cloud))
    _lib.check(ok, "houv_kd_sort")
    return (out, order) if return_order else out


def icp_refine(src, tgt, init=None, max_correspondence_distance=0.02, max_iteration=500, relative_fitness=1e-6,
               relative_rmse=1e-6):
    _lib.require_gpu(src, tgt, init)
    _want(src, _F32, "src"); _want(tgt, _F32, "tgt")
    P, N, _ = src.shape
    M = tgt.shape[1]
    if tgt.shape[0] != P or src.shape[2] != 3 or tgt.shape[2] != 3:
        raise _lib.HouvHipError("icp_refine: expected src[P,N,3], tgt[P,M,3]")
    if init is not None:
        _want(init, _F32, "init")
        if tuple(init.shape) != (P, 4, 4):
            raise _lib.HouvHipError("icp_refine: init must be [P,4,4]")
    dev = src.device
    T = torch.empty((P, 4, 4), dtype=_F32, device=dev)
    fit = torch.empty(P, dtype=_F32, device=dev)
    rmse = torch.empty(P, dtype=_F32, device=dev)
    iters = torch.empty(P, dtype=_I32, device=dev)
    with torch.cuda.device(dev):
        ok = _lib.load().houv_icp_refine(_lib.ptr(src), _lib.ptr(tgt), P, N, M, _lib.ptr(init),
                                         float(max_correspondence_distance), int(max_iteration), float(relative_fitness),
                                         float(relative_rmse), _lib.ptr(T), _lib.ptr(fit), _lib.ptr(rmse),
                                         _lib.ptr(iters), _lib.stream_of(src))
    _lib.check(ok, "houv_icp_refine")
    return dict(T=T, fitness=fit, inlier_rmse=rmse, iterations=iters)


def emd_workspace(B, N, device):
    n = _lib.load().houv_emd_workspace_bytes(int(B), int(N))
    return torch.empty(n, dtype=torch.uint8, device=device) if n > 0 else None


def emd_forward(xyz1, xyz2, eps, iters, workspace=None):
    _lib.require_gpu(xyz1.contiguous(), xyz2.contiguous())
    if xyz1.dim() != 3 or xyz2.dim() != 3 or xyz1.shape[2] != 3 or xyz2.shape[2] != 3 or xyz1.shape[0] != xyz2.shape[0]:
        raise _lib.HouvHipError("emd_forward: expected xyz1[B,N,3], xyz2[B,N,3]")
    xyz1 = xyz1.contiguous().to(_F32)
    xyz2 = xyz2.contiguous().to(_F32)
    B, N, _ = xyz1.shape
    M = xyz2.shape[1]
    dev = xyz1.device
    dist = torch.empty((B, N), dtype=_F32, device=dev)
    assignment = torch.empty((B, N), dtype=_I32, device=dev)
    iters_run = torch.empty((B,), dtype=_I32, device=dev)
    if workspace is None and N == M:
        workspace = emd_workspace(B, N, dev)
    if workspace is not None:
        _lib.require_gpu(workspace, xyz1)
        need = _lib.load().houv_emd_workspace_bytes(int(B), int(N))
        if workspace.numel() * workspace.element_size() < need:
            raise _lib.HouvHipError(f"emd_forward: the workspace holds fewer than the {need} bytes needed")
    with torch.cuda.device(dev):
        ok = _lib.load().houv_emd_forward(_lib.ptr(xyz1), _lib.ptr(xyz2), B, N, M, float(eps), int(iters), _lib.ptr(dist),
                                          _lib.ptr(assignment), _lib.ptr(iters_run), _lib.ptr(workspace),
                                          _lib.stream_of(xyz1))
    _lib.check(ok, "houv_emd_forward")
    return dist, assignment, iters_run


def emd_backward(xyz1, xyz2, graddist, assignment):
    xyz1 = xyz1.contiguous().to(_F32)
    xyz2 = xyz2.contiguous().to(_F32)
    graddist = graddist.contiguous().to(_F32)
    _lib.require_gpu(xyz1, xyz2, graddist, assignment)
    _want(assignment, _I32, "assignment")
    B, N, _ = xyz1.shape
    if xyz2.shape != xyz1.shape or graddist.numel() != B * N or assignment.numel() != B * N:
        raise _lib.HouvHipError("emd_backward: shape mismatch")
    gradxyz1 = torch.zeros_like(xyz1)
    with torch.cuda.device(xyz1.device):
        ok = _lib.load().houv_emd_backward(_lib.ptr(xyz1), _lib.ptr(xyz2), B, N, _lib.ptr(graddist), _lib.ptr(assignment),
                                           _lib.ptr(gradxyz1), _lib.stream_of(xyz1))
    _lib.check(ok, "houv_emd_backward")
    return gradxyz1


def rri_features(xyz, idx, k, skip=0):
    _lib.require_gpu(xyz, idx)
    _want(xyz, _F32, "xyz"); _want(idx, _I32, "idx")
    if xyz.dim() != 3 or xyz.shape[2] != 3 or idx.dim() != 3 or idx.shape[:2] != xyz.shape[:2]:
        raise _lib.HouvHipError("rri_features: expected xyz[B,N,3], idx[B,N,L]")
    B, N, _ = xyz.shape
    out = torch.empty((B, N, 4 * int(k)), dtype=_F32, device=xyz.device)
    with torch.cuda.device(xyz.device):
        ok = _lib.load().houv_rri_features(_lib.ptr(xyz), _lib.ptr(idx), B, N, int(k), idx.shape[2], int(skip), _lib.ptr(out),
                                           _lib.stream_of(xyz))
    _lib.check(ok, "houv_rri_features")
    return out


def gmm_params(gamma, pts):
    _lib.require_gpu(gamma, pts)
    _want(gamma, _F32, "gamma"); _want(pts, _F32, "pts")
    if gamma.dim() != 3 or pts.dim() != 3 or pts.shape[2] != 3 or pts.shape[:2] != gamma.shape[:2]:
        raise _lib.HouvHipError("gmm_params: expected gamma[B,N,J], pts[B,N,3]")
    B, N, J = gamma.shape
    pi = torch.empty((B, J), dtype=_F32, device=gamma.device)
    mu = torch.empty((B, J, 3), dtype=_F32, device=gamma.device)
    sigma = torch.empty((B, J), dtype=_F32, device=gamma.device)
    with torch.cuda.device(gamma.device):
        ok = _lib.load().houv_gmm_params(_lib.ptr(gamma), _lib.ptr(pts), B, N, J, _lib.ptr(pi), _lib.ptr(mu), _lib.ptr(sigma),
                                         _lib.stream_of(gamma))
    _lib.check(ok, "houv_gmm_params")
    return pi, mu, sigma


def gmm_register(pi_s, mu_s, mu_t, sigma_t):
    _lib.require_gpu(pi_s, mu_s, mu_t, sigma_t)
    for t, n in ((pi_s, "pi_s"), (mu_s, "mu_s"), (mu_t, "mu_t"), (sigma_t, "sigma_t")):
        _want(t, _F32, n)
    if pi_s.dim() != 2 or tuple(mu_s.shape) != tuple(pi_s.shape) + (3,) or mu_t.shape != mu_s.shape or sigma_t.shape != pi_s.shape:
        raise _lib.HouvHipError("gmm_register: expected pi_s[B,J], mu_s[B,J,3], mu_t[B,J,3], sigma_t[B,J]")
    B, J = pi_s.shape
    T = torch.empty((B, 4, 4), dtype=_F32, device=pi_s.device)
    with torch.cuda.device(pi_s.device):
        ok = _lib.load().houv_gmm_register(_lib.ptr(pi_s), _lib.ptr(mu_s), _lib.ptr(mu_t), _lib.ptr(sigma_t), B, J, _lib.ptr(T),
                                           _lib.stream_of(pi_s))
    _lib.check(ok, "houv_gmm_register")
    return T


def idam_simmat(src, tgt, es, et, W1, s1, t1, W2, b2, W3, s3, t3, w4, b4, want_rowmax=True, want_idx=True, want_corr=True,
                want_scores=False):
    par = (W1, s1, t1, W2, b2, W3, s3, t3, w4, b4)
    _lib.require_gpu(src, tgt, es, et, *par)
    for t in (src, tgt, es, et) + par:
        _want(t, _F32, "idam_simmat")
    if src.dim() != 3 or tgt.dim() != 3 or es.dim() != 3 or et.dim() != 3 or src.shape[2] != 3 or tgt.shape[2] != 3 \
            or es.shape[:2] != src.shape[:2] or et.shape[:2] != tgt.shape[:2] or tgt.shape[0] != src.shape[0] \
            or et.shape[2] != es.shape[2]:
        raise _lib.HouvHipError("idam_simmat: expected src[B,Ms,3], tgt[B,Mt,3], es[B,Ms,E], et[B,Mt,E]")
    B, Ms, E = es.shape
    Mt = tgt.shape[1]
    if tuple(W1.shape) != (32, 2 * E + 4) or tuple(W2.shape) != (32, 32) or tuple(W3.shape) != (32, 32) or b4.numel() != 1 \
            or any(t.numel() != 32 for t in (s1, t1, b2, s3, t3, w4)):
        raise _lib.HouvHipError("idam_simmat: expected W1[32,2E+4], W2[32,32], W3[32,32], b4[1] and 32-element s1, t1, b2, s3, t3, w4")
    dev = src.device
    rowmax = torch.empty((B, Ms, 32), dtype=_F32, device=dev) if want_rowmax else None
    cidx = torch.empty((B, Ms), dtype=_I32, device=dev) if want_idx else None
    corr = torch.empty((B, 3, Ms), dtype=_F32, device=dev) if want_corr else None
    scores = torch.empty((B, Ms, Mt), dtype=_F32, device=dev) if want_scores else None
    with torch.cuda.device(dev):
        ok = _lib.load().houv_idam_simmat(_lib.ptr(src), _lib.ptr(tgt), _lib.ptr(es), _lib.ptr(et), B, Ms, Mt, E,
                                          *[_lib.ptr(t) for t in par], _lib.ptr(rowmax), _lib.ptr(cidx), _lib.ptr(corr),
                                          _lib.ptr(scores), _lib.stream_of(src))
    _lib.check(ok, "houv_idam_simmat")
    return rowmax, cidx, corr, scores


def edge_diff(x, idx, k=None, ldo=None):
    _lib.require_gpu(x, idx)
    _want(x, _F32, "x"); _want(idx, _I32, "idx")
    if x.dim() != 3 or idx.dim() != 3 or idx.shape[:2] != x.shape[:2]:
        raise _lib.HouvHipError("edge_diff: expected x[B,N,C], idx[B,N,L]")
    B, N, C = x.shape
    k = idx.shape[2] if k is None else int(k)
    ldo = C if ldo is None else int(ldo)
    out = torch.empty((B * N * k, ldo), dtype=_F32, device=x.device)
    with torch.cuda.device(x.device):
        ok = _lib.load().houv_edge_diff(_lib.ptr(x), _lib.ptr(idx), B, N, k, C, idx.shape[2], ldo, _lib.ptr(out),
                                        _lib.stream_of(x))
    _lib.check(ok, "houv_edge_diff")
    return out


PCN_ROW_TILE = 64


def mlp2_max(x, W1, shift1, W2, b2, want_y=False):
    _lib.require_gpu(x, W1, shift1, W2, b2)
    for t, n in ((x, "x"), (W1, "W1"), (shift1, "shift1"), (W2, "W2"), (b2, "b2")):
        _want(t, _F32, f"mlp2_max: {n}")
    if x.dim() != 3 or W1.dim() != 2 or W2.dim() != 2 or W1.shape[1] != x.shape[2] or W2.shape[1] != W1.shape[0] \
            or b2.numel() != W2.shape[0]:
        raise _lib.HouvHipError(f"mlp2_max: expected x[B,N,Cin], W1[H,Cin], W2[Cout,H], b2[Cout], got {tuple(x.shape)}, "
                                f"{tuple(W1.shape)}, {tuple(W2.shape)}, {tuple(b2.shape)}")
    B, N, Cin = x.shape
    H, Cout = W1.shape[0], W2.shape[0]
    if tuple(shift1.shape) == (H,):
        stride = 0
    elif tuple(shift1.shape) == (B, H):
        stride = H
    else:
        raise _lib.HouvHipError(f"mlp2_max: shift1 must be [{H}] or [{B},{H}], got {tuple(shift1.shape)}")
    dev = x.device
    pooled = torch.empty((B, Cout), dtype=_F32, device=dev)
    y = torch.empty((B, N, Cout), dtype=_F32, device=dev) if want_y else None
    lib = _lib.load()
    nbytes = lib.houv_mlp2_max_workspace_bytes(B, N, Cout)
    ws = torch.empty(nbytes // 4, dtype=_F32, device=dev) if nbytes > 0 else None
    with torch.cuda.device(dev):
        ok = lib.houv_mlp2_max(_lib.ptr(x), B, N, Cin, _lib.ptr(W1), H, _lib.ptr(shift1), stride, _lib.ptr(W2), _lib.ptr(b2),
                               Cout, _lib.ptr(pooled), _lib.ptr(y), _lib.ptr(ws), _lib.stream_of(x))
    _lib.check(ok, "houv_mlp2_max")
    return pooled, y


def mlp2_max_arg(x, W1, shift1, W2, b2, want_y=False):
    _lib.require_gpu(x, W1, shift1, W2, b2)
    for t, n in ((x, "x"), (W1, "W1"), (shift1, "shift1"), (W2, "W2"), (b2, "b2")):
        _want(t, _F32, f"mlp2_max_arg: {n}")
    if x.dim() != 3 or W1.dim() != 2 or W2.dim() != 2 or W1.shape[1] != x.shape[2] or W2.shape[1] != W1.shape[0] \
            or b2.numel() != W2.shape[0]:
        raise _lib.HouvHipError(f"mlp2_max_arg: expected x[B,N,Cin], W1[H,Cin], W2[Cout,H], b2[Cout], got {tuple(x.shape)}, "
                                f"{tuple(W1.shape)}, {tuple(W2.shape)}, {tuple(b2.shape)}")
    B, N, Cin = x.shape
    H, Cout = W1.shape[0], W2.shape[0]
    if tuple(shift1.shape) == (H,):
        stride = 0
    elif tuple(shift1.shape) == (B, H):
        stride = H
    else:
        raise _lib.HouvHipError(f"mlp2_max_arg: shift1 must be [{H}] or [{B},{H}], got {tuple(shift1.shape)}")
    dev = x.device
    pooled = torch.empty((B, Cout), dtype=_F32, device=dev)
    arg = torch.empty((B, Cout), dtype=_I32, device=dev)
    y = torch.empty((B, N, Cout), dtype=_F32, device=dev) if want_y else None
    lib = _lib.load()
    nbytes = lib.houv_mlp2_max_arg_workspace_bytes(B, N, Cout)
    ws = torch.empty(nbytes // 4, dtype=_F32, device=dev) if nbytes > 0 else None
    with torch.cuda.device(dev):
        ok = lib.houv_mlp2_max_arg(_lib.ptr(x), B, N, Cin, _lib.ptr(W1), H, _lib.ptr(shift1), stride, _lib.ptr(W2), _lib.ptr(b2),
                                   Cout, _lib.ptr(pooled), _lib.ptr(arg), _lib.ptr(y), _lib.ptr(ws), _lib.stream_of(x))
    _lib.check(ok, "houv_mlp2_max_arg")
    return pooled, arg, y


def mlp2_max_backward(x, W1, shift1, W2, arg, gpooled, rows=None, nrows=None, gy_rows=None, want_gx=False):
    ts = (x, W1, shift1, W2, gpooled)
    _lib.require_gpu(*ts, arg)
    for t, n in zip(ts, ("x", "W1", "shift1", "W2", "gpooled")):
        _want(t, _F32, f"mlp2_max_backward: {n}")
    _want(arg, _I32, "mlp2_max_backward: arg")
    if x.dim() != 3 or W1.dim() != 2 or W2.dim() != 2 or W1.shape[1] != x.shape[2] or W2.shape[1] != W1.shape[0]:
        raise _lib.HouvHipError(f"mlp2_max_backward: expected x[B,N,Cin], W1[H,Cin], W2[Cout,H], got {tuple(x.shape)}, "
                                f"{tuple(W1.shape)}, {tuple(W2.shape)}")
    B, N, Cin = x.shape
    H, Cout = W1.shape[0], W2.shape[0]
    if tuple(arg.shape) != (B, Cout) or tuple(gpooled.shape) != (B, Cout):
        raise _lib.HouvHipError(f"mlp2_max_backward: arg and gpooled must be [{B},{Cout}], got {tuple(arg.shape)}, {tuple(gpooled.shape)}")
    if tuple(shift1.shape) == (H,):
        stride = 0
    elif tuple(shift1.shape) == (B, H):
        stride = H
    else:
        raise _lib.HouvHipError(f"mlp2_max_backward: shift1 must be [{H}] or [{B},{H}], got {tuple(shift1.shape)}")
    R = 0
    if rows is not None or nrows is not None or gy_rows is not None:
        if rows is None or nrows is None or gy_rows is None:
            raise _lib.HouvHipError("mlp2_max_backward: rows, nrows and gy_rows come together")
        _lib.require_gpu(rows, nrows, gy_rows)
        _want(rows, _I32, "mlp2_max_backward: rows"); _want(nrows, _I32, "mlp2_max_backward: nrows")
        _want(gy_rows, _F32, "mlp2_max_backward: gy_rows")
        if rows.dim() != 2 or rows.shape[0] != B or tuple(nrows.shape) != (B,) or tuple(gy_rows.shape) != (B, rows.shape[1], Cout):
            raise _lib.HouvHipError(f"mlp2_max_backward: expected rows[{B},R], nrows[{B}], gy_rows[{B},R,{Cout}], got "
                                    f"{tuple(rows.shape)}, {tuple(nrows.shape)}, {tuple(gy_rows.shape)}")
        R = rows.shape[1]
        if R == 0:
            rows = nrows = gy_rows = None
    dev = x.device
    lib = _lib.load()
    rcap = lib.houv_mlp2_max_backward_rows(N, Cout, R)
    out = dict(gW1=torch.empty((H, Cin), dtype=_F32, device=dev), gshift1=torch.empty((B, H), dtype=_F32, device=dev),
               gW2=torch.empty((Cout, H), dtype=_F32, device=dev), gb2=torch.empty((Cout,), dtype=_F32, device=dev),
               act_rows=torch.empty((B, rcap), dtype=_I32, device=dev), nact=torch.empty((B,), dtype=_I32, device=dev),
               gx_rows=torch.empty((B, rcap, Cin), dtype=_F32, device=dev) if want_gx else None)
    nbytes = lib.houv_mlp2_max_backward_workspace_bytes(B, N, Cin, H, Cout, R)
    ws = torch.empty(max(nbytes, 16) // 4, dtype=_F32, device=dev)
    with torch.cuda.device(dev):
        ok = lib.houv_mlp2_max_backward(_lib.ptr(x), B, N, Cin, _lib.ptr(W1), H, _lib.ptr(shift1), stride, _lib.ptr(W2), Cout,
                                        _lib.ptr(arg), _lib.ptr(gpooled), _lib.ptr(rows), _lib.ptr(nrows), _lib.ptr(gy_rows), R,
                                        _lib.ptr(out["gW1"]), _lib.ptr(out["gshift1"]), _lib.ptr(out["gW2"]), _lib.ptr(out["gb2"]),
                                        _lib.ptr(out["act_rows"]), _lib.ptr(out["nact"]), _lib.ptr(out["gx_rows"]), _lib.ptr(ws),
                                        _lib.stream_of(x))
    _lib.check(ok, "houv_mlp2_max_backward")
    return out


def pcn_fold(coarse, cvec, grid, Wgp, W2, b2, W3, b3):
    ts = (coarse, cvec, grid, Wgp, W2, b2, W3, b3)
    _lib.require_gpu(*ts)
# ... 614 lines not shown
```

houv_amd/solver.py:

```python
import os

import numpy as np
import weakref

import torch

from . import ops

RETRY_THRESHOLD = 0.030
ITERS_PER_LAUNCH = 50

LAUNCH_LOG = None

LATTICE_AXES = np.array([(x, y, z) for x in (-1, 0, 1) for y in (-1, 0, 1) for z in (-1, 0, 1)
                         if (x, y, z) != (0, 0, 0)], dtype=np.float64)


def houv_init_params(n_inst, seed=2021):
    np.random.seed(seed)
    V = np.random.randn(n_inst, 3)
    if n_inst < 26:
        raise IndexError(f"index {n_inst} is out of bounds for axis 0 with size {n_inst}")
    V[:26] = LATTICE_AXES
    np.random.seed(seed)
    a = np.random.randn(n_inst, 1)
    np.random.seed(seed)
    c = np.random.randn(n_inst, 3)
    np.random.seed(seed)
    s = np.random.randn(n_inst, 1)
    return np.concatenate([V, a, c, s], axis=1).astype(np.float32).astype(np.float64)


def solve_twin_init_params(n_inst):
    V = np.random.randn(n_inst, 3)
    a = np.random.randn(n_inst, 1)
    c = np.random.randn(n_inst, 3)
    s = np.random.randn(n_inst, 1)
    np.random.randn(n_inst, 3)
    return np.concatenate([V, a, c, s], axis=1)


PRUNED = os.environ.get("HOUV_SOLVER", "pruned").strip().lower() != "brute"
PRUNED_MAX_POINTS = 4096
PRUNED_MIN_POINTS = 257


def uses_pruned(N, M, pruned=None):
    pruned = PRUNED if pruned is None else pruned
    return bool(pruned) and PRUNED_MIN_POINTS <= max(N, M) <= PRUNED_MAX_POINTS


def morton_sort(cloud):
    lo = cloud.min(dim=1, keepdim=True)[0]
    hi = cloud.max(dim=1, keepdim=True)[0]
    q = ((cloud - lo) / (hi - lo + 1e-9) * 1023.0).to(torch.int64).clamp_(0, 1023)

    def spread(x):
        x = (x | (x << 16)) & 0x030000FF
        x = (x | (x << 8)) & 0x0300F00F
        x = (x | (x << 4)) & 0x030C30C3
        x = (x | (x << 2)) & 0x09249249
        return x
    code = spread(q[..., 0]) | (spread(q[..., 1]) << 1) | (spread(q[..., 2]) << 2)
    order = torch.argsort(code, dim=1, stable=True)
    return torch.gather(cloud, 1, order.unsqueeze(2).expand(-1, -1, 3)).contiguous()


KD_RULE = "area"


def _split_segments(seg, cut, rule):
    S, L, _ = seg.shape
    if rule == "area":
        best = out = None
        for ax in range(3):
            o = torch.argsort(seg[..., ax], dim=1, stable=True)
            cand = torch.gather(seg, 1, o.unsqueeze(2).expand(-1, -1, 3))

            def area(x):
                e = x.max(dim=1)[0] - x.min(dim=1)[0]
                return e[:, 0] * e[:, 1] + e[:, 1] * e[:, 2] + e[:, 0] * e[:, 2]
            cost = area(cand[:, :cut]) + area(cand[:, cut:])
            if best is None:
                best, out = cost, cand
            else:
                take = cost < best
                best = torch.where(take, cost, best)
                out = torch.where(take.view(S, 1, 1), cand, out)
        return out
    ext = seg.max(dim=1)[0] - seg.min(dim=1)[0]
    axis = ext.argmax(dim=1)
    key = torch.gather(seg, 2, axis.view(S, 1, 1).expand(-1, L, 1))[..., 0]
    order = torch.argsort(key, dim=1, stable=True)
    return torch.gather(seg, 1, order.unsqueeze(2).expand(-1, -1, 3))


def kd_sort(cloud, leaf=32, rule=None):
    P, N, _ = cloud.shape
    rule = rule or KD_RULE
    for ax in (2, 1, 0):
        order = torch.argsort(cloud[..., ax], dim=1, stable=True)
        cloud = torch.gather(cloud, 1, order.unsqueeze(2).expand(-1, -1, 3))
    segs = [(0, N)]
    while True:
        nxt, groups = [], {}
        for (a, b) in segs:
            tiles = -(-(b - a) // leaf)
            if tiles <= 1:
                nxt.append((a, b))
                continue
            mid = a + (tiles - tiles // 2) * leaf
            groups.setdefault((b - a, mid - a), []).append(a)
            nxt += [(a, mid), (mid, b)]
        if not groups:
            break
        for (length, cut), starts in groups.items():
            if len(starts) == 1:
                a = starts[0]
                cloud[:, a:a + length] = _split_segments(cloud[:, a:a + length], cut, rule)
            else:
                idx = (torch.tensor(starts, device=cloud.device).view(-1, 1) + torch.arange(length, device=cloud.device).view(1, -1)).reshape(-1)
                seg = cloud[:, idx].reshape(P * len(starts), length, 3)
                cloud[:, idx] = _split_segments(seg, cut, rule).reshape(P, len(starts) * length, 3)
        segs = nxt
    return cloud.contiguous()


SPATIAL_SORT = "kd"
KD_SORT_IMPL = os.environ.get("HOUV_KD_SORT", "hip").strip().lower()
KD_SORT_HIP_MAX_POINTS = 4096


def _kd_sort_on_device(cloud):
    return (KD_SORT_IMPL == "hip" and SPATIAL_SORT == "kd" and KD_RULE in ops.KD_RULES and cloud.is_cuda
            and cloud.dtype == torch.float32 and cloud.dim() == 3 and cloud.shape[2] == 3
            and 1 <= cloud.shape[1] <= KD_SORT_HIP_MAX_POINTS)


_SORTED = {}


def spatial_sort(cloud, leaf=32):
    if _sorted_leaf(cloud) == leaf:
        return cloud
    if _kd_sort_on_device(cloud):
        out = ops.kd_sort(cloud.contiguous(), leaf, KD_RULE)
    else:
        out = kd_sort(cloud, leaf) if SPATIAL_SORT == "kd" else morton_sort(cloud)
    _mark_sorted(out, leaf)
    return out


def sort_leaf(N, M):
    return 32 if max(N, M) <= 2048 else 64


def _sorted_leaf(cloud):
    m = _SORTED.get(cloud.data_ptr()) if cloud.is_contiguous() else None
    ok = m is not None and m[5]() is cloud and m[:4] == (cloud._version, tuple(cloud.shape), cloud.device, SPATIAL_SORT + KD_RULE)
    return m[4] if ok else None


def _mark_sorted(cloud, leaf):
    if len(_SORTED) > 512:
        for key in [k for k, v in _SORTED.items() if v[5]() is None]:
            del _SORTED[key]
        if len(_SORTED) > 512:
            _SORTED.clear()
    _SORTED[cloud.data_ptr()] = (cloud._version, tuple(cloud.shape), cloud.device, SPATIAL_SORT + KD_RULE, leaf, weakref.ref(cloud))


FUSED_MAX_POINTS = 4096

LARGE_IMPL = os.environ.get("HOUV_LARGE", "fused").strip().lower()
LARGE_MIN_POINTS = 4097
LARGE_MAX_POINTS = 16384
LARGE_LAUNCH_BUDGET_S = 0.25
LARGE_PAIRS_PER_S_PER_CU = 18e9
LARGE_CHUNK = 4096


def uses_large(N, M):
    return LARGE_IMPL == "fused" and LARGE_MIN_POINTS <= max(N, M) <= LARGE_MAX_POINTS


def large_launch_seconds(hypotheses, iters, N, M, n_cu):
    pad = lambda x: -(-x // LARGE_CHUNK) * LARGE_CHUNK
    per_round = (pad(N) * M + pad(M) * N) / LARGE_PAIRS_PER_S_PER_CU
    return -(-hypotheses // n_cu) * iters * per_round


def large_launch_plan(P, K, N, M, n_cu, budget_s=None):
    budget = LARGE_LAUNCH_BUDGET_S if budget_s is None else budget_s
    rounds = max(1, int(budget / large_launch_seconds(1, 1, N, M, n_cu)))
    pairs = max(1, min(P, rounds * n_cu // K))
    waves = -(-pairs * K // n_cu)
    return pairs, max(1, min(ITERS_PER_LAUNCH, rounds // waves))


def _run_stage_large(src, tgt, p, K, n_iters, *, angle_base, trans_mode, use_views, f64_params, lr, iters_per_launch,
                     want_grad, want_cd, alpha, want_last_params):
    from . import _lib
    _lib.require_gpu(src, tgt)
    P, N, _ = src.shape
    M = tgt.shape[1]
    dev = src.device
    n = P * K
    state = torch.zeros((n, 24), dtype=torch.float64, device=dev)
    state[:, :8] = p.to(dev)
    k_full, k_view = int(N * alpha), int(N * 1)
    pairs, step = large_launch_plan(P, K, N, M, torch.cuda.get_device_properties(dev).multi_processor_count)
    if iters_per_launch:
        step = min(step, iters_per_launch)
    last_params = torch.empty((n, 8), dtype=torch.float64, device=dev) if want_last_params else None
    outs = []
    for p0 in range(0, P, pairs):
        p1 = min(P, p0 + pairs)
        rows = slice(p0 * K, p1 * K)
        s_src, s_tgt, s_state = src[p0:p1], tgt[p0:p1], state[rows]
        done, out = 0, None
        while done < n_iters:
            it = min(step, n_iters - done)
            if want_last_params:
                if done == n_iters - 1:
                    last_params[rows] = s_state[:, :8]
                else:
                    it = min(it, n_iters - 1 - done)
            last = done + it == n_iters
            if LAUNCH_LOG is not None:
                ev0 = torch.cuda.Event(enable_timing=True)
                ev1 = torch.cuda.Event(enable_timing=True)
                ev0.record(torch.cuda.current_stream(dev))
            out = ops.solve_iterate(s_src, s_tgt, s_state, K, steps_done=done, n_iters=it, angle_base=angle_base,
                                    trans_mode=trans_mode, use_views=use_views, f64_params=f64_params, k_full=k_full,
                                    k_view=k_view, lr=lr, loss_scale=1.0 / n, want_grad=want_grad and last,
                                    want_cd=want_cd and last, large=True)
            if LAUNCH_LOG is not None:
                ev1.record(torch.cuda.current_stream(dev))
                LAUNCH_LOG.append((ev0, ev1, (p1 - p0) * K, it, N, M, bool(use_views), False, done == 0))
            done += it
        outs.append(out)
    out = outs[0] if len(outs) == 1 else {key: torch.cat([o[key] for o in outs]) for key in outs[0]}
    if want_last_params:
        out["last_params"] = last_params
    return out, state


def _run_stage_unfused(src, tgt, params, K, n_iters, *, angle_base, trans_mode, use_views, f64_params, lr, want_grad,
                       want_cd, alpha):
    import math
    from .model_utils_completion import calc_cd_percent, loss_view
    from .train_utils import rotation, translation
    dev = src.device
    P, N, _ = src.shape
    n = P * K
    dt = torch.float64 if f64_params else torch.float32
    p0 = torch.as_tensor(params, dtype=torch.float64).to(dev)
    leaves = [p0[:, 0:3].to(dt).clone().requires_grad_(True), p0[:, 3:4].to(dt).clone().requires_grad_(True),
              p0[:, 4:7].to(dt).clone().requires_grad_(True), p0[:, 7:8].to(dt).clone().requires_grad_(True)]
    opt = torch.optim.Adam(leaves, lr=lr)
    srck = src.repeat_interleave(K, dim=0)
    tgtk = tgt.repeat_interleave(K, dim=0)
    out = None
    for it in range(n_iters):
        V, a, c, sc = (l.float() for l in leaves)
        angle = torch.sin(a * math.pi) * math.pi / 8 + math.pi / 8 + angle_base * math.pi / 4
        R = rotation(angle, V)
        sigma = torch.sin(sc * math.pi) * 0.125 + 0.125 if trans_mode == 0 else torch.sin(sc * math.pi)
        T = translation(c, sigma)
        moved = torch.bmm(srck, R.transpose(1, 2)) + T
        cds = [calc_cd_percent(moved, tgtk, percent=alpha)]
        min_1, _ = torch.min(torch.stack(cds[0], dim=1), dim=1)
        loss = min_1 * 6
        if use_views:
            for d in range(3):
                cds.append(loss_view(moved, tgtk, dim=d))
                v, _ = torch.min(torch.stack(cds[-1], dim=1), dim=1)
                loss = loss + v
        opt.zero_grad()
        loss.mean().backward()
        if it == n_iters - 1:
            out = dict(score=min_1.detach().float(), loss=loss.detach().float(), R=R.detach().float().contiguous(),
                       T=T.detach().float()[:, 0].contiguous(),
                       last_params=torch.cat([l.detach() for l in leaves], dim=1).double())
            if want_grad:
                out["grad"] = torch.cat([l.grad for l in leaves], dim=1).float()
            if want_cd:
                cd = torch.zeros((n, 8), dtype=torch.float32, device=dev)
                for m, (c0, c1) in enumerate(cds):
                    cd[:, 2 * m], cd[:, 2 * m + 1] = c0.detach(), c1.detach()
                out["cd"] = cd
        opt.step()
    state = torch.zeros((n, 24), dtype=torch.float64, device=dev)
    state[:, :8] = torch.cat([l.detach() for l in leaves], dim=1).double()
    state[:, 8:16] = torch.cat([opt.state[l]["exp_avg"] for l in leaves], dim=1).double()
    state[:, 16:24] = torch.cat([opt.state[l]["exp_avg_sq"] for l in leaves], dim=1).double()
    return out, state


def run_stage(src, tgt, params, K, n_iters, *, angle_base, trans_mode, use_views, f64_params, lr,
              iters_per_launch=None, want_grad=False, want_cd=False, alpha=0.5, pruned=None, want_last_params=False):
    if n_iters < 1:
        raise ValueError("num_epochs must be >= 1 (the reference reads the last iteration's outputs)")
    src = src.contiguous().float()
    tgt = tgt.contiguous().float()
    P, N, _ = src.shape
    if use_views and tgt.shape[1] != N:
        raise RuntimeError(f"The size of tensor a ({tgt.shape[1]}) must match the size of tensor b ({N}) at "
                           "non-singleton dimension 1")
    dev = src.device
    n = P * K
    p = torch.as_tensor(params, dtype=torch.float64)
    if tuple(p.shape) != (n, 8):
        raise ValueError(f"params must be [{n},8]")
    if uses_large(N, tgt.shape[1]):
        return _run_stage_large(src, tgt, p, K, n_iters, angle_base=angle_base, trans_mode=trans_mode, use_views=use_views,
                                f64_params=f64_params, lr=lr, iters_per_launch=iters_per_launch, want_grad=want_grad,
                                want_cd=want_cd, alpha=alpha, want_last_params=want_last_params)
    if max(N, tgt.shape[1]) > FUSED_MAX_POINTS:
        from . import _lib
        _lib.require_gpu(src, tgt)
        return _run_stage_unfused(src, tgt, p, K, n_iters, angle_base=angle_base, trans_mode=trans_mode,
                                  use_views=use_views, f64_params=f64_params, lr=lr, want_grad=want_grad,
                                  want_cd=want_cd, alpha=alpha)
    state = torch.zeros((n, 24), dtype=torch.float64, device=dev)
    state[:, :8] = p.to(dev)
    k_full = int(N * alpha)
    k_view = int(N * 1)
    step = iters_per_launch or ITERS_PER_LAUNCH
    pruned = PRUNED if pruned is None else pruned
    nn_ws = None
    if uses_pruned(N, tgt.shape[1], pruned):
        leaf = sort_leaf(N, tgt.shape[1])
        src, tgt = spatial_sort(src, leaf), spatial_sort(tgt, leaf)
        nn_ws = ops.solve_workspace(n, N, tgt.shape[1], dev)
    done, out = 0, None
    last_params = None
    while done < n_iters:
        it = min(step, n_iters - done)
        if want_last_params:
            if done == n_iters - 1:
                last_params = state[:, :8].clone()
            else:
                it = min(it, n_iters - 1 - done)
        last = done + it == n_iters
        if LAUNCH_LOG is not None:
            ev0 = torch.cuda.Event(enable_timing=True)
            ev1 = torch.cuda.Event(enable_timing=True)
            ev0.record(torch.cuda.current_stream(dev))
        out = ops.solve_iterate(src, tgt, state, K, steps_done=done, n_iters=it, angle_base=angle_base,
                                trans_mode=trans_mode, use_views=use_views, f64_params=f64_params, k_full=k_full,
                                k_view=k_view, lr=lr, loss_scale=1.0 / n, want_grad=want_grad and last,
                                want_cd=want_cd and last, nn_ws=nn_ws,
                                ws_valid="verify" if pruned == "verify" else done > 0)
        if LAUNCH_LOG is not None:
            ev1.record(torch.cuda.current_stream(dev))
            LAUNCH_LOG.append((ev0, ev1, n, it, N, tgt.shape[1], bool(use_views), nn_ws is not None, done == 0))
        done += it
    if want_last_params:
        out["last_params"] = last_params
    return out, state


CONCURRENT_RETRIES = True
_retry_streams = {}


def _side_streams(dev):
    key = (dev.type, dev.index)
    if key not in _retry_streams:
        _retry_streams[key] = [torch.cuda.Stream(device=dev) for _ in range(3)]
    return _retry_streams[key]


def best_of_k_with_retry(stage_fn, src, tgt):
    B = src.shape[0]
    score, R, T = stage_fn(src, tgt, 0)
    best, _ = score.topk(1, dim=1, largest=False, sorted=True)
    retry = torch.nonzero(best[:, 0] > RETRY_THRESHOLD).reshape(-1)
    if retry.numel() > 0:
        s_add, t_add = src[retry].contiguous(), tgt[retry].contiguous()
        for sub, whole in ((s_add, src), (t_add, tgt)):
            leaf = _sorted_leaf(whole)
            if leaf is not None:
                _mark_sorted(sub, leaf)
        outs = {}
        if CONCURRENT_RETRIES and src.is_cuda:
            main = torch.cuda.current_stream(src.device)
            side = _side_streams(src.device)
            for base in range(1, 4):
                side[base - 1].wait_stream(main)
                with torch.cuda.stream(side[base - 1]):
                    outs[base] = stage_fn(s_add, t_add, base)
            for base in range(1, 4):
                main.wait_stream(side[base - 1])
                for x in outs[base]:
                    x.record_stream(main)
            s_add.record_stream(side[0]); s_add.record_stream(side[1]); s_add.record_stream(side[2])
            t_add.record_stream(side[0]); t_add.record_stream(side[1]); t_add.record_stream(side[2])
        else:
            for base in range(1, 4):
                outs[base] = stage_fn(s_add, t_add, base)
        for base in range(1, 4):
            score_a, R_a, T_a = outs[base]
            best_a, _ = score_a.topk(1, dim=1, largest=False, sorted=True)
            flag = torch.nonzero((best_a < best[retry]).reshape(-1)).reshape(-1)
            ge = retry[flag]
            R[ge] = R_a[flag]
            score[ge] = score_a[flag]
            T[ge] = T_a[flag]
            best[ge] = best_a[flag]
    _, k = score.topk(1, dim=1, largest=False, sorted=True)
    pick = k[:, 0]
    rows = torch.arange(B, device=score.device)
    ans = torch.zeros((B, 4, 4), dtype=torch.float32, device=score.device)
    ans[:, :3, :3] = R[rows, pick]
    ans[:, :3, 3] = T[rows, pick]
    return ans, score, retry
```

include/houv_hip.h:

```cpp
#ifndef HOUV_HIP_H_
#define HOUV_HIP_H_

#include <stdint.h>

#ifdef __cplusplus
extern "C" {
#endif

#define HOUV_ABI_VERSION 2

int houv_abi_version(void);

const char* houv_last_error(void);

const char* houv_build_id(void);

int houv_debug_set(const char* name, long long value);

int houv_chamfer_forward(const float* xyz1, const float* xyz2, int B, int N, int M,
                         float* dist1, float* dist2, int32_t* idx1, int32_t* idx2, void* stream);

int houv_chamfer_backward(const float* xyz1, const float* xyz2, int B, int N, int M,
                          const float* graddist1, const float* graddist2,
                          const int32_t* idx1, const int32_t* idx2,
                          float* gradxyz1, float* gradxyz2, void* stream);

int houv_kabsch(const float* src, const float* corr, const float* w_or_null, int B, int N,
                float* R, float* t, void* stream);

int houv_solve_iterate(const float* src, const float* tgt, int P, int N, int M, int K,
                       double* state, int steps_done, int n_iters,
                       int angle_base, int trans_mode, int use_views, int f64_params,
                       int k_full, int k_view,
                       double lr, double beta1, double beta2, double eps, float loss_scale,
                       float* out_score, float* out_loss, float* out_R, float* out_T,
                       float* out_grad, float* out_cd, void* stream);

int houv_solve_iterate_pruned(const float* src, const float* tgt, int P, int N, int M, int K,
                              double* state, int steps_done, int n_iters,
                              int angle_base, int trans_mode, int use_views, int f64_params,
                              int k_full, int k_view,
                              double lr, double beta1, double beta2, double eps, float loss_scale,
                              float* out_score, float* out_loss, float* out_R, float* out_T,
                              float* out_grad, float* out_cd,
                              int16_t* nn_ws, int ws_valid, int ws_stride, void* stream);

#define HOUV_LARGE_MAX_POINTS 16384
int houv_solve_iterate_large(const float* src, const float* tgt, int P, int N, int M, int K,
                             double* state, int steps_done, int n_iters,
                             int angle_base, int trans_mode, int use_views, int f64_params,
                             int k_full, int k_view,
                             double lr, double beta1, double beta2, double eps, float loss_scale,
                             float* out_score, float* out_loss, float* out_R, float* out_T,
                             float* out_grad, float* out_cd, void* stream);

int houv_solve_variant(int N, int M, int pruned, int* block, int* points_per_lane, int* prune_mode);

long long houv_solve_lds_bytes(int N, int M, int pruned);

int houv_solve_walk_variant(int need);

int houv_kd_sort(const float* xyz, int P, int N, int leaf, int rule, float* out, int32_t* order_or_null, void* stream);

int houv_icp_refine(const float* src, const float* tgt, int P, int N, int M, const float* init_or_null,
                    float max_correspondence_distance, int max_iteration, float relative_fitness,
                    float relative_rmse, float* out_T, float* out_fitness, float* out_rmse, int32_t* out_iters,
                    void* stream);


int houv_knn(const float* xyz, int B, int N, int k, int32_t* idx, void* stream);

int houv_edgeconv1(const float* xyz, const int32_t* idx, int B, int N, int k, const float* W, const float* scale,
                   const float* shift, float* out, void* stream);

int houv_max_over_k(const float* act, long long npts, int k, int C, float* out, int ldo, void* stream);

int houv_gemm_f32(const float* A, const float* B, float* C, int M, int N, int K, int lda, int ldb, int ldc,
                  int trans_b, int outer, int inner, long long sAo, long long sAi, long long sBo, long long sBi,
                  long long sCo, long long sCi, float alpha, const float* scale_or_null, const float* shift_or_null,
                  const float* residual_or_null, int ldr, long long sRo, long long sRi, int relu, void* stream);

int houv_attention_f32(const float* Q, const float* K, const float* V, float* O, int P, int H, int Nq, int Nk, int dk,
                       int ldq, int ldk, int ldv, int ldo, long long sQ, long long sK, long long sV, long long sO,
                       float scale, void* stream);

int houv_layernorm(const float* x, long long rows, int D, const float* a, const float* b, float eps,
                   const float* residual_or_null, float* out, void* stream);

int houv_softmax_rows(float* x, long long rows, int L, void* stream);

int houv_softmax_corr(const float* scores, int P, int N, int M, const float* pts, float* corr, void* stream);


int houv_furthest_point_sample(const float* xyz, int B, int N, int npoint, int32_t* idx, void* stream);

int houv_knn_cross(const float* query, const float* ref, int B, int N, int M, int k, float* dist2, int32_t* idx,
                   void* stream);

int houv_gather_points(const float* features, const int32_t* idx, int B, int C, int N, int M, float* out, void* stream);

int houv_ball_query(const float* xyz, const float* center, int B, int N, int Mc, float min_radius, float max_radius,
                    int nsample, int32_t* idx, int32_t* cnt_or_null, void* stream);

int houv_three_interpolate(const float* features, const int32_t* idx, const float* weight, int B, int C, int M, int N,
                           float* out, void* stream);

int houv_scatter_points_grad(const float* grad_out, const int32_t* idx, const float* weight_or_null, int B, int C, int N,
                             int M, int S, float* grad_features, void* workspace, void* stream);

long long houv_scatter_points_workspace_bytes(int B, int N, int M);

int houv_emd_forward(const float* xyz1, const float* xyz2, int B, int N, int M, float eps, int iters, float* dist,
                     int32_t* assignment, int32_t* iters_run_or_null, void* workspace_or_null, void* stream);

long long houv_emd_workspace_bytes(int B, int N);

int houv_emd_backward(const float* xyz1, const float* xyz2, int B, int N, const float* graddist, const int32_t* assignment,
                      float* gradxyz1, void* stream);


int houv_rri_features(const float* xyz, const int32_t* idx, int B, int N, int k, int idx_ld, int idx_skip, float* out,
                      void* stream);

int houv_gmm_params(const float* gamma, const float* pts, int B, int N, int J, float* pi, float* mu, float* sigma,
                    void* stream);

int houv_gmm_register(const float* pi_s, const float* mu_s, const float* mu_t, const float* sigma_t, int B, int J, float* T,
                      void* stream);


int houv_idam_simmat(const float* src, const float* tgt, const float* es, const float* et, int B, int Ms, int Mt, int E,
                     const float* W1, const float* s1, const float* t1, const float* W2, const float* b2, const float* W3,
                     const float* s3, const float* t3, const float* w4, const float* b4, float* rowmax_or_null,
                     int32_t* corr_idx_or_null, float* corr_or_null, float* scores_or_null, void* stream);

int houv_edge_diff(const float* X, const int32_t* idx, int B, int N, int k, int C, int idx_ld, int ldo, float* out,
                   void* stream);


#define HOUV_PCN_ROW_TILE 64

int houv_mlp2_max(const float* x, int B, int N, int Cin, const float* W1, int H, const float* shift1, long long shift1_stride,
                  const float* W2, const float* b2, int Cout, float* pooled, float* y_or_null, float* workspace, void* stream);
long long houv_mlp2_max_workspace_bytes(int B, int N, int Cout);

int houv_mlp2_max_arg(const float* x, int B, int N, int Cin, const float* W1, int H, const float* shift1,
                      long long shift1_stride, const float* W2, const float* b2, int Cout, float* pooled, int32_t* arg,
                      float* y_or_null, float* workspace, void* stream);
long long houv_mlp2_max_arg_workspace_bytes(int B, int N, int Cout);

int houv_mlp2_max_backward(const float* x, int B, int N, int Cin, const float* W1, int H, const float* shift1,
                           long long shift1_stride, const float* W2, int Cout, const int32_t* arg, const float* gpooled,
                           const int32_t* rows_or_null, const int32_t* nrows_or_null, const float* gy_rows_or_null, int R,
                           float* gW1, float* gshift1, float* gW2, float* gb2, int32_t* act_rows, int32_t* nact,
                           float* gx_rows_or_null, void* workspace, void* stream);
long long houv_mlp2_max_backward_workspace_bytes(int B, int N, int Cin, int H, int Cout, int R);
int houv_mlp2_max_backward_rows(int N, int Cout, int R);

int houv_pcn_fold(const float* coarse, const float* cvec, const float* grid, int B, int nc, int scale, const float* Wgp,
                  const float* W2, const float* b2, const float* W3, const float* b3, float* fine, void* stream);

int houv_pcn_fold_backward(const float* coarse, const float* cvec, const float* grid, int B, int nc, int scale, const float* Wgp,
                           const float* W2, const float* b2, const float* W3, const float* b3, const float* gfine,
                           float* gcoarse, float* gcvec, float* gWgp, float* gW2, float* gb2, float* gW3, float* gb3,
                           void* workspace, long long workspace_bytes, void* stream);
long long houv_pcn_fold_backward_workspace_bytes(int B, int nc, int scale);


#define HOUV_KNN_FEAT_BLOCK 32
#define HOUV_KNN_FEAT_CHUNK 16
#define HOUV_DENSE_CONV_GROWTH 24

int houv_knn_feat(const float* x, int B, int N, int C, int ldx, int k, int32_t* idx, float* dist2_or_null, void* stream);

int houv_dense_conv(const float* x, int ldx, const int32_t* idx, int B, int N, int C, int k, const float* W0, const float* b0,
                    const float* W1, const float* b1, const float* W2, const float* b2, int relu_out, float* out, int ldo,
                    void* stream);

int houv_dense_conv_arg(const float* x, int ldx, const int32_t* idx, int B, int N, int C, int k, const float* W0, const float* b0,
                        const float* W1, const float* b1, const float* W2, const float* b2, int relu_out, float* out, int ldo,
                        int8_t* arg, void* stream);

int houv_dense_conv_backward(const float* x, int ldx, const int32_t* idx, int B, int N, int C, int k, const float* W0,
                             const float* b0, const float* W1, const float* b1, const float* W2, const float* b2, int relu_out,
                             const int8_t* arg, const float* out_or_null, int ldo, const float* gout, int ldg, float* gx, int ldgx,
                             float* gW0, float* gb0, float* gW1, float* gb1, float* gW2, float* gb2, void* workspace,
                             long long workspace_bytes, void* stream);
long long houv_dense_conv_backward_workspace_bytes(int B, int N, int C, int k);


#define HOUV_SA_ATTN_BLOCK 128

int houv_sa_attn(const float* P, int ldp, const float* x, int ldx, const int32_t* idx, int B, int N, int C, int k,
                 const float* Ww1, const float* Ww2, const float* bw2, const float* Wout, const float* bout, int relu_out,
                 float* out, int ldo, void* stream);

int houv_sa_attn_backward(const float* P, int ldp, const int32_t* idx, int B, int N, int C, int k, const float* Ww1,
                          const float* Ww2, const float* bw2, const float* G, int ldg, float* gP, int ldgp, float* ro, int ldro,
                          float* gWw1, float* gWw2, float* gbw2, void* workspace, long long workspace_bytes, void* stream);
long long houv_sa_attn_backward_workspace_bytes(int B, int N, int C, int k);

int houv_edge_pool(const float* feat, int ldx, const int32_t* p_idx, const int32_t* pn_idx, int B, int N, int S, int C, int pk,
                   float* out, int ldo, int8_t* arg_or_null, void* stream);

int houv_edge_pool_backward(const float* g, int ldg, const int32_t* p_idx, const int32_t* pn_idx, const int8_t* arg, int B, int N,
                            int S, int C, int pk, float* gfeat, int ldgx, void* workspace, long long workspace_bytes, void* stream);
long long houv_edge_pool_backward_workspace_bytes(int B, int N, int S, int pk);

int houv_ef_expand(const float* proj, int ldp, const int32_t* idx, int B, int N, int O, int k, int r, const float* W2a, int ldw,
                   const float* W3, const float* b3, float* out, int ldo, int8_t* arg_or_null, void* stream);

int houv_ef_expand_backward(const float* proj, int ldp, const int32_t* idx, const int8_t* arg, int B, int N, int O, int k, int r,
                            const float* W2a, int ldw, const float* W3, const float* g, int ldg, float* gproj, int ldgp,
                            float* gW2a, float* gW3, float* gb3, void* workspace, long long workspace_bytes, void* stream);
long long houv_ef_expand_backward_workspace_bytes(int B, int N, int O, int k, int r);

int houv_pose_forward(const float* params, int n, int angle_base, int trans_mode,
                      const float* src_or_null, int N, float* R, float* T, float* moved_or_null, void* stream);

#ifdef __cplusplus
}
#endif
#endif
```

Baseline: 214.9 pairs/s.

## Run solve stage as one persistent-grid launch with atomic chunk work queue

Replaces the sequence of per-chunk solve launches (ITERS_PER_LAUNCH iterations each) with a single persistent kernel launch. Workgroups pull (chunk, hypothesis) items from an atomic counter and spin-wait on a per-hypothesis done flag before continuing the next chunk. This is meant to remove launch gaps and tail-idle time between chunks and to let workgroups flow across chunks. In exchange it adds polling, atomics, a timeout path that invalidates results, and a host-side status check.

```diff
diff --git a/houv_amd/_lib.py b/houv_amd/_lib.py
--- a/houv_amd/_lib.py
+++ b/houv_amd/_lib.py
@@ -29,6 +29,12 @@
     "houv_solve_iterate_pruned": (ctypes.c_int, [_c_f, _c_f, _int, _int, _int, _int, _c_f, _int, _int, _int, _int, _int,
                                                  _int, _int, _int, _dbl, _dbl, _dbl, _dbl, _flt, _c_f, _c_f, _c_f, _c_f,
                                                  _c_f, _c_f, _c_f, _int, _int, _c_f]),
+    "houv_solve_stage": (ctypes.c_int, [_c_f, _c_f, _int, _int, _int, _int, _c_f, _int, _int, _int, _int, _int, _int,
+                                        _int, _int, _dbl, _dbl, _dbl, _dbl, _flt, _c_f, _c_f, _c_f, _c_f, _c_f, _c_f,
+                                        _int, _c_f, _c_f]),
+    "houv_solve_stage_pruned": (ctypes.c_int, [_c_f, _c_f, _int, _int, _int, _int, _c_f, _int, _int, _int, _int, _int,
+                                               _int, _int, _int, _dbl, _dbl, _dbl, _dbl, _flt, _c_f, _c_f, _c_f, _c_f,
+                                               _c_f, _c_f, _c_f, _int, _int, _int, _c_f, _c_f]),
     "houv_solve_variant": (ctypes.c_int, [_int, _int, _int, ctypes.POINTER(ctypes.c_int), ctypes.POINTER(ctypes.c_int),
                                           ctypes.POINTER(ctypes.c_int)]),
     "houv_solve_lds_bytes": (ctypes.c_longlong, [_int, _int, _int]),
diff --git a/houv_amd/csrc/capi.hip b/houv_amd/csrc/capi.hip
--- a/houv_amd/csrc/capi.hip
+++ b/houv_amd/csrc/capi.hip
@@ -58,7 +58,8 @@
   using namespace houv;
   const struct { const char* name; std::atomic<int>* knob; long long lo, hi, step; } ints[] = {
       {"solve_predict", &g_debug.pred_mode, 0, 2, 1}, {"knn_split", &g_debug.knn_split, 0, 1, 1},
-      {"attn_split", &g_debug.attn_split, 0, 1, 1},   {"gemm_split", &g_debug.gemm_split, 0, 6, 3}};
+      {"attn_split", &g_debug.attn_split, 0, 1, 1},   {"gemm_split", &g_debug.gemm_split, 0, 6, 3},
+      {"solve_max_workgroups", &g_debug.max_workgroups, 0, 0x7fffffff, 1}};
   if (name && !strcmp(name, "solve_stats")) {
     g_debug.stats = (unsigned long long)value;
     return 1;
@@ -69,6 +70,10 @@
   }
   if (name && !strcmp(name, "solve_cull_stats")) {
     g_debug.cull_stats = (unsigned long long)value;
+    return 1;
+  }
+  if (name && !strcmp(name, "solve_sched")) {
+    g_debug.sched = (unsigned long long)value;
     return 1;
   }
   for (const auto& k : ints)
diff --git a/houv_amd/csrc/houv_common.h b/houv_amd/csrc/houv_common.h
--- a/houv_amd/csrc/houv_common.h
+++ b/houv_amd/csrc/houv_common.h
@@ -32,6 +32,8 @@
   std::atomic<unsigned long long> stats{0ull};
   std::atomic<unsigned long long> walk_hist{0ull};
   std::atomic<unsigned long long> cull_stats{0ull};
+  std::atomic<unsigned long long> sched{0ull};
+  std::atomic<int> max_workgroups{0};
   std::atomic<int> knn_split{1};
   std::atomic<int> attn_split{1};
   std::atomic<int> gemm_split{6};
diff --git a/houv_amd/csrc/houv_math.h b/houv_amd/csrc/houv_math.h
--- a/houv_amd/csrc/houv_math.h
+++ b/houv_amd/csrc/houv_math.h
@@ -416,4 +416,14 @@
   }
 }
 
-}
+HOUV_HD inline int sched_chunks(int n_iters, int chunk_iters) { return (n_iters - 1) / chunk_iters + 1; }
+HOUV_HD inline long long sched_items64(int ninst, int n_iters, int chunk_iters) {
+  return (long long)ninst * sched_chunks(n_iters, chunk_iters);
+}
+HOUV_HD inline int sched_items(int ninst, int n_iters, int chunk_iters) { return ninst * sched_chunks(n_iters, chunk_iters); }
+HOUV_HD inline int sched_item_iters(int n_iters, int chunk_iters, int chunk) {
+  const int left = n_iters - chunk * chunk_iters;
+  return left < chunk_iters ? left : chunk_iters;
+}
+
+}
diff --git a/houv_amd/csrc/solve.hip b/houv_amd/csrc/solve.hip
--- a/houv_amd/csrc/solve.hip
+++ b/houv_amd/csrc/solve.hip
@@ -16,11 +16,23 @@
   unsigned long long* stats;
   unsigned long long* walk_hist;
   unsigned long long* cull_stats;
+  int* sched_ws;
+  int chunk_iters;
+  unsigned long long* sched;
 };
 
 constexpr int kRescanBatch = 4;
 constexpr int kRefresh = 4;
 constexpr int kTermMaxAge = 0;
+constexpr unsigned long long kPollTicksPerIter = 2000000ull;
+
+constexpr int kItemSteps = 0, kItemIters = 1, kItemWsValid = 2, kItemInst = 3, kItemClk = 4;
+
+__device__ __forceinline__ int xcc_id() {
+  int v;
+  asm volatile("s_getreg_b32 %0, hwreg(HW_REG_XCC_ID)" : "=s"(v));
+  return v & 7;
+}
 
 struct Smem {
   float4* tgt;
@@ -321,17 +333,70 @@
   constexpr int TS = (PRUNE == 3) ? 1 : 0;
   constexpr int kPad = kSub << TS;
   extern __shared__ __attribute__((aligned(512))) unsigned char smem_raw[];
+  if (fresh(a.sched) && tid_x() == 0) {
+    int* ctl = carve(smem_raw, a.N, a.M, BLOCK, PRUNE ? BLOCK * Q : 0, kPad).ctl;
+    const unsigned long long t0 = __builtin_amdgcn_s_memrealtime();
+    ctl[2] = (int)(unsigned)t0;
+    ctl[3] = (int)(unsigned)(t0 >> 32);
+    ctl[4] = 0;
+  }
+#pragma unroll 1
+  for (;;) {
   const int N = a.N, M = a.M;
   const Smem sm = carve(smem_raw, N, M, BLOCK, PRUNE ? BLOCK * Q : 0, kPad);
   const int tid = tid_x();
   const int ninst = a.P * a.K;
-  int inst = blockIdx.x;
-  if ((ninst & 7) == 0) inst = (blockIdx.x & 7) * (ninst >> 3) + (blockIdx.x >> 3);
+  int inst = blockIdx.x, steps_done = a.steps_done, n_iters = a.n_iters, ws_valid = a.ws_valid, chunk = 0;
+  if (a.sched_ws) {
+    if (tid == 0) {
+      int t = atomicAdd(a.sched_ws, 1);
+      const int c = t / ninst;
+      if (t < sched_items(ninst, a.n_iters, a.chunk_iters) && c > 0) {
+        const int* done = a.sched_ws + 4 + (t - c * ninst);
+        const unsigned long long t0 = __builtin_amdgcn_s_memrealtime();
+        const unsigned long long limit = (unsigned long long)fresh(a.n_iters) * kPollTicksPerIter;
+        while (__hip_atomic_load(done, __ATOMIC_RELAXED, __HIP_MEMORY_SCOPE_AGENT) < c) {
+          if (__builtin_amdgcn_s_memrealtime() - t0 > limit) {
+            __hip_atomic_store(a.sched_ws + 1, 1, __ATOMIC_RELAXED, __HIP_MEMORY_SCOPE_AGENT);
+            t = 0x7fffffff;
+            break;
+          }
+          __builtin_amdgcn_s_sleep(32);
+        }
+        __builtin_amdgcn_fence(__ATOMIC_ACQUIRE, "agent");
+        asm volatile("s_waitcnt vmcnt(0)" ::: "memory");
+      }
+      sm.ctl[1] = t;
+    }
+    __syncthreads();
+    const int t = __builtin_amdgcn_readfirstlane(sm.ctl[1]);
+    if (t >= sched_items(ninst, a.n_iters, a.chunk_iters)) break;
+    chunk = t / ninst;
+    inst = t - chunk * ninst;
+    steps_done = a.steps_done + chunk * a.chunk_iters;
+    n_iters = sched_item_iters(a.n_iters, a.chunk_iters, chunk);
+    ws_valid = (a.ws_valid != 0 || chunk > 0) ? 1 : 0;
+    if (fresh(a.sched) && tid == 0) sm.ctl[4] += 1;
+  } else {
+    if ((ninst & 7) == 0) inst = (blockIdx.x & 7) * (ninst >> 3) + (blockIdx.x >> 3);
+    if (fresh(a.sched) && tid == 0) sm.ctl[4] = 1;
+  }
+  int* const iw = PRUNE ? reinterpret_cast<int*>(sm.anchor + kAnchorFloats) : sm.ctl + 8 + BLOCK / 64;
+  if (tid == 0) {
+    iw[kItemSteps] = steps_done;
+    iw[kItemIters] = n_iters;
+    iw[kItemWsValid] = ws_valid;
+    iw[kItemInst] = inst;
+  }
+  auto item = [&](int i) {
+    return __builtin_amdgcn_readfirstlane(*reinterpret_cast<const int*>(fresh_lds(reinterpret_cast<const float*>(iw + i))));
+  };
   const int pair = inst / a.K;
   const buf_t src = make_buf(a.src + (size_t)pair * N * 3, N * 12);
   const float* __restrict__ tgt = a.tgt + (size_t)pair * M * 3;
   const int npad = (N + kPad - 1) / kPad * kPad, mpad = (M + kPad - 1) / kPad * kPad;
-  const float4 pad4 = make_float4(INFINITY, INFINITY, INFINITY, 0.f);
+  const float inf = __uint_as_float(fresh(0x7f800000u));
+  const float4 pad4 = make_float4(inf, inf, inf, 0.f);
 
   for (int j = tid; j < mpad; j += BLOCK) sm.tgt[j] = (j < M) ? make_float4(tgt[j * 3], tgt[j * 3 + 1], tgt[j * 3 + 2], 0.f) : pad4;
   for (int j = N + tid; j < npad; j += BLOCK) sm.mov[j] = pad4;
@@ -363,12 +428,12 @@
 #pragma unroll
     for (int k = 0; k < 8; ++k) p[k] = (float)sm.state[k];
     Pose f;
-    pose_forward(p, a.angle_base, a.trans_mode, f);
+    pose_forward(p, fresh(a.angle_base), fresh(a.trans_mode), f);
     store_pose(sm.pose, f);
   }
   if (tid == kAdamTid) {
-    const int step = a.steps_done + 1;
-    const AdamScalars asc = adam_scalars(step, a.lr, a.beta1, a.beta2);
+    const int step = steps_done + 1;
+    const AdamScalars asc = adam_scalars(step, fresh(a.lr), fresh(a.beta1), fresh(a.beta2));
     sm.adam[(step & 1) * 2 + 0] = asc.step_size;
     sm.adam[(step & 1) * 2 + 1] = asc.bc2_sqrt;
   }
@@ -381,9 +446,8 @@
       const float v = __builtin_fmaf(z, z, __builtin_fmaf(y, y, x * x));
       r2 = (v <= r2) ? r2 : ((v < INFINITY) ? v : INFINITY);
     }
-#pragma unroll
-    for (int o = 1; o < 64; o <<= 1) r2 = fmaxf(r2, __shfl_xor(r2, o, 64));
-    if ((tid & 63) == 0) sm.red[tid >> 6] = r2;
+    r2 = wave_fmax_to_lane63(r2);
+    if ((tid & 63) == 63) sm.red[tid >> 6] = r2;
     if (tid == 0) {
       sm.ctl[0] = (int)(((1u << NMET) - 1u) * 0x11u);
       reinterpret_cast<unsigned*>(sm.anchor)[kTermAges] = 0u;
@@ -398,19 +462,21 @@
     }
   }
 
-  unsigned long long clk0 = 0ull, rt0 = 0ull;
-  if (a.stats) {
-    clk0 = __builtin_amdgcn_s_memtime();
-    rt0 = __builtin_amdgcn_s_memrealtime();
+  if (a.stats && tid == 0) {
+    const unsigned long long clk0 = __builtin_amdgcn_s_memtime(), rt0 = __builtin_amdgcn_s_memrealtime();
+    iw[kItemClk] = (int)(unsigned)clk0;
+    iw[kItemClk + 1] = (int)(unsigned)(clk0 >> 32);
+    iw[kItemClk + 2] = (int)(unsigned)rt0;
+    iw[kItemClk + 3] = (int)(unsigned)(rt0 >> 32);
   }
   constexpr int NW = BLOCK / 64;
   constexpr unsigned kAllMet = (1u << NMET) - 1u;
   unsigned pred_a = kAllMet;
   auto red_row = [&](int dir) { return sm.red + ((size_t)dir * NW + (tid_x() >> 6)) * kRedStride; };
 #pragma unroll 1
-  for (int it = 0; it < a.n_iters; ++it) {
+  for (int it = 0; it < item(kItemIters); ++it) {
     if (a.pred_mode == 1) pred_a = 0u;
-    const bool allgrad = a.pred_mode == 2 || ((PRUNE != 0) && (((a.steps_done + it) % kRefresh) == 0 || (a.ws_valid == 0 && it == 0)));
+    const bool allgrad = a.pred_mode == 2 || ((PRUNE != 0) && (((item(kItemSteps) + it) % kRefresh) == 0 || (it == 0 && item(kItemWsValid) == 0)));
     unsigned need_a = kAllMet, need_b = kAllMet;
     if constexpr (PRUNE != 0) {
       const unsigned w = (unsigned)__builtin_amdgcn_readfirstlane(*reinterpret_cast<const int*>(fresh_lds(reinterpret_cast<const float*>(sm.ctl))));
@@ -436,7 +502,7 @@
       int btile[Q][NMET];
       if constexpr (PRUNE) {
         tile_boxes<BLOCK, Q, TS>(mx, my, mz, N, npad / kPad, sm.mbox);
-        pruned_now = (a.ws_valid != 0) || (it > 0);
+        pruned_now = (it > 0) || (item(kItemWsValid) != 0);
       }
       if (need_a != 0u) {
         if (pruned_now) {
@@ -445,7 +511,7 @@
                                                 need_a, sm.st, ws_res, best, btile, a.stats, fresh(a.walk_hist), fresh(a.cull_stats));
         } else {
           sweep<Q, NMET>(sm.tgt, mpad / kTrk, mx, my, mz, best, btile);
-          if (a.stats && (tid & 63) == 0) atomicAdd(&a.stats[3], 1ull);
+          if (a.stats && (tid_x() & 63) == 0) atomicAdd(&a.stats[3], 1ull);
         }
         unsigned sel[NMET];
         select_all<BLOCK, Q, NMET>(sm, best, N, a.k_full, a.k_view, need_a, hrot, sel);
@@ -465,7 +531,7 @@
         const float4 v = (i < M) ? sm.tgt[i] : make_float4(0.f, 0.f, 0.f, 0.f);
         tx[k] = v.x; ty[k] = v.y; tz[k] = v.z;
       }
-      const bool pruned_now = (PRUNE != 0) && ((a.ws_valid != 0) || (it > 0));
+      const bool pruned_now = (PRUNE != 0) && ((it > 0) || (item(kItemWsValid) != 0));
       auto pick_winners = [&]() {
         __syncthreads();
         final_sums<BLOCK, NMET>(sm, 0, true, 0u, need_b);
@@ -483,7 +549,7 @@
                                                 need_b, sm.st, ws_res, best, btile, a.stats, fresh(a.walk_hist), fresh(a.cull_stats));
         } else {
           sweep<Q, NMET>(sm.mov, npad / kTrk, tx, ty, tz, best, btile);
-          if (a.stats && (tid & 63) == 0) atomicAdd(&a.stats[3], 1ull);
+          if (a.stats && (tid_x() & 63) == 0) atomicAdd(&a.stats[3], 1ull);
         }
         unsigned sel[NMET];
         select_all<BLOCK, Q, NMET>(sm, best, M, a.k_full, a.k_view, need_b, hrot, sel);
@@ -511,13 +577,13 @@
     static_assert(NMET * kAccN <= 64, "final_sums runs on the scalar tail's wave");
     __builtin_amdgcn_wave_barrier();
 
-    if (kAdamTid != 0 && tid == kAdamTid && it + 1 < a.n_iters) {
-      const int step = a.steps_done + it + 2;
+    if (kAdamTid != 0 && tid_x() == kAdamTid && it + 1 < iw[kItemIters]) {
+      const int step = iw[kItemSteps] + it + 2;
       const AdamScalars asc = adam_scalars(step, fresh(a.lr), fresh(a.beta1), fresh(a.beta2));
       sm.adam[(step & 1) * 2 + 0] = asc.step_size;
       sm.adam[(step & 1) * 2 + 1] = asc.bc2_sqrt;
     }
-    if (tid == 0) {
+    if (tid_x() == 0) {
       const int k_full = fresh(a.k_full), k_view = fresh(a.k_view);
       const float loss_scale = fresh(a.loss_scale);
       const double lr = fresh(a.lr), beta1 = fresh(a.beta1), beta2 = fresh(a.beta2), eps = fresh(a.eps);
@@ -526,8 +592,8 @@
       load_pose(f, sm.pose);
       TailLoss r;
       solve_tail_loss<NMET>(sm.acc, kAccStride, f, k_full, k_view, loss_scale, trans_mode, r);
-      if (it == a.n_iters - 1)
-        store_outputs(a.out_score, a.out_loss, a.out_R, a.out_T, a.out_grad, a.out_cd, inst, f, r);
+      if (iw[kItemSteps] + it == fresh(a.steps_done) + fresh(a.n_iters) - 1)
+        store_outputs(a.out_score, a.out_loss, a.out_R, a.out_T, a.out_grad, a.out_cd, iw[kItemInst], f, r);
       if constexpr (PRUNE != 0) {
 #pragma unroll
         for (int m = 0; m < NMET; ++m) {
@@ -535,12 +601,12 @@
           if ((need_a >> m) & 1u) sm.anchor[2 * m + 1] = r.cd[m][1];
         }
       }
-      const int step = a.steps_done + it + 1;
+      const int step = iw[kItemSteps] + it + 1;
       const AdamScalars asc{sm.adam[(step & 1) * 2 + 0], sm.adam[(step & 1) * 2 + 1]};
       solve_tail_step(r.g, sm.state, a.f64_params, asc, beta1, beta2, eps, angle_base, trans_mode, f);
       if constexpr (PRUNE != 0) {
         unsigned next = kAllMet | (kAllMet << 4), ages = 0u;
-        const bool all_next = fresh(a.pred_mode) == 2 || it + 2 >= a.n_iters;
+        const bool all_next = fresh(a.pred_mode) == 2 || it + 2 >= iw[kItemIters];
         if (!all_next) {
           const unsigned have = need_b | (need_a << 4);
           float* stale = reinterpret_cast<float*>(sm.tbox) + 3;
@@ -571,7 +637,7 @@
         }
       }
       store_pose(sm.pose, f);
-      if (kAdamTid == 0 && it + 1 < a.n_iters) {
+      if (kAdamTid == 0 && it + 1 < iw[kItemIters]) {
         const AdamScalars nxt = adam_scalars(step + 1, lr, beta1, beta2);
         sm.adam[((step + 1) & 1) * 2 + 0] = nxt.step_size;
         sm.adam[((step + 1) & 1) * 2 + 1] = nxt.bc2_sqrt;
@@ -579,31 +645,76 @@
     }
     __syncthreads();
   }
-  if (tid_x() < 24) a.state[(size_t)inst * 24 + tid_x()] = sm.state[tid_x()];
-  if (a.stats) {
-    const unsigned long long dc = __builtin_amdgcn_s_memtime() - clk0, dr = __builtin_amdgcn_s_memrealtime() - rt0;
-    if (tid == 0) {
-      atomicAdd(&a.stats[4], dc);
-      atomicAdd(&a.stats[5], dr);
-    }
-  }
+  if (tid_x() < 24) a.state[(size_t)item(kItemInst) * 24 + tid_x()] = sm.state[tid_x()];
+  if (a.stats && tid_x() == 0) {
+    const unsigned long long clk0 = (unsigned long long)(unsigned)iw[kItemClk] | ((unsigned long long)(unsigned)iw[kItemClk + 1] << 32);
+    const unsigned long long rt0 = (unsigned long long)(unsigned)iw[kItemClk + 2] | ((unsigned long long)(unsigned)iw[kItemClk + 3] << 32);
+    atomicAdd(&a.stats[4], __builtin_amdgcn_s_memtime() - clk0);
+    atomicAdd(&a.stats[5], __builtin_amdgcn_s_memrealtime() - rt0);
+  }
+  if (!fresh(a.sched_ws)) break;
+  asm volatile("s_waitcnt vmcnt(0)" ::: "memory");
+  __syncthreads();
+  if (tid_x() == 0) {
+    const int t = sm.ctl[1], c = t / ninst;
+    __builtin_amdgcn_fence(__ATOMIC_RELEASE, "agent");
+    asm volatile("s_waitcnt vmcnt(0)" ::: "memory");
+    __hip_atomic_store(a.sched_ws + 4 + (t - c * ninst), c + 1, __ATOMIC_RELAXED, __HIP_MEMORY_SCOPE_AGENT);
+  }
+  }
+  if (fresh(a.sched) && tid_x() == 0) {
+    unsigned long long* s = fresh(a.sched) + 4 * xcc_id();
+    const int* ctl = carve(smem_raw, a.N, a.M, BLOCK, PRUNE ? BLOCK * Q : 0, kPad).ctl;
+    const unsigned long long t0 = (unsigned long long)(unsigned)ctl[2] | ((unsigned long long)(unsigned)ctl[3] << 32);
+    const unsigned long long t1 = __builtin_amdgcn_s_memrealtime();
+    atomicAdd(s + 0, (unsigned long long)ctl[4]);
+    atomicAdd(s + 1, t1 - t0);
+    atomicMin(s + 2, t0);
+    atomicMax(s + 3, t1);
+  }
+}
+
+template <typename Kernel>
+int stage_grid(Kernel kernel, const SolveArgs& a, int block, size_t bytes, const char* who) {
+  int dev = 0, cus = 0, per_cu = 0;
+  hipError_t e = hipGetDevice(&dev);
+  if (e == hipSuccess) e = hipDeviceGetAttribute(&cus, hipDeviceAttributeMultiprocessorCount, dev);
+  if (e == hipSuccess) e = hipOccupancyMaxActiveBlocksPerMultiprocessor(&per_cu, kernel, block, bytes);
+  if (e != hipSuccess || cus < 1 || per_cu < 1) {
+    set_error("%s: cannot size the persistent grid (%d CUs x %d workgroups): %s", who, cus, per_cu, hipGetErrorString(e));
+    return 0;
+  }
+  long long grid = (long long)cus * per_cu;
+  if (grid > (long long)a.P * a.K) grid = (long long)a.P * a.K;
+  const int cap = g_debug.max_workgroups.load();
+  if (cap > 0 && grid > cap) grid = cap;
+  if (sched_items64(a.P * a.K, a.n_iters, a.chunk_iters) + grid > 0x7fffffffLL) {
+    set_error("%s: too many (hypothesis, chunk) items for one stage", who);
+    return 0;
+  }
+  return (int)grid;
+}
+
+template <typename Kernel>
+int launch_kernel(Kernel kernel, const SolveArgs& a, int block, size_t bytes, hipStream_t s, const char* who) {
+  hipError_t e = hipFuncSetAttribute((const void*)kernel, hipFuncAttributeMaxDynamicSharedMemorySize, (int)bytes);
+  if (e != hipSuccess) { set_error("%s: cannot reserve %zu B of LDS: %s", who, bytes, hipGetErrorString(e)); return 0; }
+  int grid = a.P * a.K;
+  if (a.sched_ws) {
+    grid = stage_grid(kernel, a, block, bytes, who);
+    if (grid < 1) return 0;
+    e = hipMemsetAsync(a.sched_ws, 0, (4 + (size_t)a.P * a.K) * sizeof(int), s);
+    if (e != hipSuccess) { set_error("%s: cannot zero sched_ws: %s", who, hipGetErrorString(e)); return 0; }
+  }
+  kernel<<<grid, block, bytes, s>>>(a);
+  return check_launch(who) ? 1 : 0;
 }
 
 template <int BLOCK, int Q, int PRUNE>
-int launch(const SolveArgs& a, int use_views, hipStream_t s) {
+int launch(const SolveArgs& a, int use_views, hipStream_t s, const char* who) {
   const size_t bytes = smem_bytes(a.N, a.M, BLOCK, PRUNE, Q);
-  const int grid = a.P * a.K;
-  hipError_t e;
-  if (use_views) {
-    e = hipFuncSetAttribute((const void*)solve_kernel<BLOCK, Q, 4, PRUNE>, hipFuncAttributeMaxDynamicSharedMemorySize, (int)bytes);
-    if (e != hipSuccess) { set_error("houv_solve_iterate: cannot reserve %zu B of LDS: %s", bytes, hipGetErrorString(e)); return 0; }
-    solve_kernel<BLOCK, Q, 4, PRUNE><<<grid, BLOCK, bytes, s>>>(a);
-  } else {
-    e = hipFuncSetAttribute((const void*)solve_kernel<BLOCK, Q, 1, PRUNE>, hipFuncAttributeMaxDynamicSharedMemorySize, (int)bytes);
-    if (e != hipSuccess) { set_error("houv_solve_iterate: cannot reserve %zu B of LDS: %s", bytes, hipGetErrorString(e)); return 0; }
-    solve_kernel<BLOCK, Q, 1, PRUNE><<<grid, BLOCK, bytes, s>>>(a);
-  }
-  return check_launch("houv_solve_iterate") ? 1 : 0;
+  if (use_views) return launch_kernel(solve_kernel<BLOCK, Q, 4, PRUNE>, a, BLOCK, bytes, s, who);
+  return launch_kernel(solve_kernel<BLOCK, Q, 1, PRUNE>, a, BLOCK, bytes, s, who);
 }
 
 }
@@ -679,15 +790,25 @@
 }
 
 static int solve_dispatch(const houv::SolveCommon& c, int use_views, short* nn_ws, int ws_valid, int ws_stride, bool prune,
-                          void* stream, const char* who) {
+                          void* stream, const char* who, bool stage = false, int chunk_iters = 0, int32_t* sched_ws = nullptr) {
   using namespace houv;
   const int ok = solve_check_args(who, c, use_views);
   if (ok < 2) return ok;
+  if (stage && chunk_iters < 1) {
+    set_error("%s: chunk_iters must be >= 1, got %d", who, chunk_iters);
+    return 0;
+  }
+  if (stage && (!sched_ws || ((uintptr_t)sched_ws & 3))) {
+    set_error("%s: sched_ws must be a 4-byte aligned int32 [4 + P*K] on the device", who);
+    return 0;
+  }
   const int N = c.N, M = c.M;
   SolveArgs a{c, nn_ws, ws_valid, ws_stride, g_debug.pred_mode.load(),
               reinterpret_cast<unsigned long long*>(g_debug.stats.load()),
               reinterpret_cast<unsigned long long*>(g_debug.walk_hist.load()),
-              reinterpret_cast<unsigned long long*>(g_debug.cull_stats.load())};
+              reinterpret_cast<unsigned long long*>(g_debug.cull_stats.load()),
+              stage ? sched_ws : nullptr, stage ? chunk_iters : 0,
+              reinterpret_cast<unsigned long long*>(g_debug.sched.load())};
   hipStream_t s = (hipStream_t)stream;
   const int mx = N > M ? N : M;
   int block = 0, q = 0, mode = 0;
@@ -707,15 +828,15 @@
   if (mode == 0) a.nn_ws = nullptr;
 #define HOUV_GO(B_, Q_)                                                          \
   if (block == B_ && q == Q_) {                                                  \
-    if (mode == 2) return launch<B_, Q_, ((B_ >= 256 && Q_ >= 2) ? 2 : 0)>(a, use_views, s);    \
-    return launch<B_, Q_, 0>(a, use_views, s);                                   \
+    if (mode == 2) return launch<B_, Q_, ((B_ >= 256 && Q_ >= 2) ? 2 : 0)>(a, use_views, s, who);    \
+    return launch<B_, Q_, 0>(a, use_views, s, who);                                   \
   }
   if (mx <= 2048) {
     HOUV_GO(64, 1) HOUV_GO(128, 1) HOUV_GO(256, 1) HOUV_GO(256, 2) HOUV_GO(256, 3) HOUV_GO(256, 4)
     HOUV_GO(512, 3) HOUV_GO(512, 4)
   } else {
-    if (block == 1024 && q == 3) return mode == 3 ? launch<1024, 3, 3>(a, use_views, s) : launch<1024, 3, 0>(a, use_views, s);
-    if (block == 1024 && q == 4) return mode == 3 ? launch<1024, 4, 3>(a, use_views, s) : launch<1024, 4, 0>(a, use_views, s);
+    if (block == 1024 && q == 3) return mode == 3 ? launch<1024, 3, 3>(a, use_views, s, who) : launch<1024, 3, 0>(a, use_views, s, who);
+    if (block == 1024 && q == 4) return mode == 3 ? launch<1024, 4, 3>(a, use_views, s, who) : launch<1024, 4, 0>(a, use_views, s, who);
   }
 #undef HOUV_GO
   set_error("%s: no kernel variant <%d,%d>", who, block, q);
@@ -742,3 +863,25 @@
                             lr, beta1, beta2, eps, loss_scale, out_score, out_loss, out_R, out_T, out_grad, out_cd};
   return solve_dispatch(a, use_views, (short*)nn_ws, ws_valid, ws_stride, true, stream, "houv_solve_iterate_pruned");
 }
+
+extern "C" int houv_solve_stage(const float* src, const float* tgt, int P, int N, int M, int K, double* state, int steps_done,
+                                int n_iters, int angle_base, int trans_mode, int use_views, int f64_params, int k_full,
+                                int k_view, double lr, double beta1, double beta2, double eps, float loss_scale,
+                                float* out_score, float* out_loss, float* out_R, float* out_T, float* out_grad, float* out_cd,
+                                int chunk_iters, int32_t* sched_ws, void* stream) {
+  const houv::SolveCommon a{src, tgt, P, N, M, K, state, steps_done, n_iters, angle_base, trans_mode, f64_params, k_full, k_view,
+                            lr, beta1, beta2, eps, loss_scale, out_score, out_loss, out_R, out_T, out_grad, out_cd};
+  return solve_dispatch(a, use_views, nullptr, 0, 0, false, stream, "houv_solve_stage", true, chunk_iters, sched_ws);
+}
+
+extern "C" int houv_solve_stage_pruned(const float* src, const float* tgt, int P, int N, int M, int K, double* state,
+                                       int steps_done, int n_iters, int angle_base, int trans_mode, int use_views,
+                                       int f64_params, int k_full, int k_view, double lr, double beta1, double beta2,
+                                       double eps, float loss_scale, float* out_score, float* out_loss, float* out_R,
+                                       float* out_T, float* out_grad, float* out_cd, int16_t* nn_ws, int ws_valid,
+                                       int ws_stride, int chunk_iters, int32_t* sched_ws, void* stream) {
+  const houv::SolveCommon a{src, tgt, P, N, M, K, state, steps_done, n_iters, angle_base, trans_mode, f64_params, k_full, k_view,
+                            lr, beta1, beta2, eps, loss_scale, out_score, out_loss, out_R, out_T, out_grad, out_cd};
+  return solve_dispatch(a, use_views, (short*)nn_ws, ws_valid, ws_stride, true, stream, "houv_solve_stage_pruned", true,
+                        chunk_iters, sched_ws);
+}
diff --git a/houv_amd/ops.py b/houv_amd/ops.py
--- a/houv_amd/ops.py
+++ b/houv_amd/ops.py
@@ -86,8 +86,8 @@
 
 def solve_iterate_out(src, tgt, state, K, steps_done, n_iters, angle_base, trans_mode, use_views, f64_params, k_full,
                       k_view, lr, beta1, beta2, eps, loss_scale, out_score, out_loss, out_R, out_T, out_grad=None,
-                      out_cd=None, nn_ws=None, ws_valid=0, large=False):
-    _lib.require_gpu(src, tgt, state, out_score, out_loss, out_R, out_T, out_grad, out_cd, nn_ws)
+                      out_cd=None, nn_ws=None, ws_valid=0, large=False, chunk_iters=None, sched_ws=None):
+    _lib.require_gpu(src, tgt, state, out_score, out_loss, out_R, out_T, out_grad, out_cd, nn_ws, sched_ws)
     _want(src, _F32, "src"); _want(tgt, _F32, "tgt"); _want(state, _F64, "state")
     P, N, _ = src.shape
     M = tgt.shape[1]
@@ -108,9 +108,23 @@
               _lib.ptr(out_loss), _lib.ptr(out_R), _lib.ptr(out_T), _lib.ptr(out_grad), _lib.ptr(out_cd))
     if large and nn_ws is not None:
         raise _lib.HouvHipError("solve_iterate: the large-cloud kernel is a brute-force sweep and takes no workspace")
+    stage = sched_ws is not None
+    if stage:
+        if large:
+            raise _lib.HouvHipError("solve_iterate: the large-cloud kernel has no stage form")
+        if sched_ws.dtype != torch.int32 or sched_ws.numel() < 4 + n:
+            raise _lib.HouvHipError(f"solve_iterate: sched_ws must hold {4 + n} int32 (ops.solve_sched_workspace)")
+        sched = (int(chunk_iters), _lib.ptr(sched_ws))
     with torch.cuda.device(src.device):
         if large:
             ok = _lib.load().houv_solve_iterate_large(*common, _lib.stream_of(src))
+        elif stage and nn_ws is None:
+            ok = _lib.load().houv_solve_stage(*common, *sched, _lib.stream_of(src))
+        elif stage:
+            if nn_ws.dtype != torch.int16 or nn_ws.dim() != 3 or tuple(nn_ws.shape[:2]) != (n, 16) or not nn_ws.is_contiguous():
+                raise _lib.HouvHipError("solve_iterate: nn_ws must be a contiguous int16 [P*K,16,stride] tensor (ops.solve_workspace)")
+            ok = _lib.load().houv_solve_stage_pruned(*common, _lib.ptr(nn_ws), int(ws_valid), nn_ws.shape[2], *sched,
+                                                     _lib.stream_of(src))
         elif nn_ws is None:
             ok = _lib.load().houv_solve_iterate(*common, _lib.stream_of(src))
         else:
@@ -118,7 +132,8 @@
                 raise _lib.HouvHipError("solve_iterate: nn_ws must be a contiguous int16 [P*K,16,stride] tensor (ops.solve_workspace)")
             ok = _lib.load().houv_solve_iterate_pruned(*common, _lib.ptr(nn_ws), int(ws_valid), nn_ws.shape[2],
                                                        _lib.stream_of(src))
-    _lib.check(ok, "houv_solve_iterate" + ("_large" if large else "_pruned" if nn_ws is not None else ""))
+    _lib.check(ok, ("houv_solve_stage" if stage else "houv_solve_iterate") +
+               ("_large" if large else "_pruned" if nn_ws is not None else ""))
     return 1
 
 
@@ -135,9 +150,13 @@
     return torch.empty((int(n_hypotheses), 16, stride), dtype=torch.int16, device=device)
 
 
+def solve_sched_workspace(n_hypotheses, device):
+    return torch.empty(4 + int(n_hypotheses), dtype=torch.int32, device=device)
+
+
 def solve_iterate(src, tgt, state, K, *, steps_done, n_iters, angle_base, trans_mode, use_views, f64_params, k_full,
                   k_view, lr, loss_scale, betas=(0.9, 0.999), eps=1e-8, want_grad=False, want_cd=False, nn_ws=None,
-                  ws_valid=False, large=False):
+                  ws_valid=False, large=False, chunk_iters=None, sched_ws=None):
     _lib.require_gpu(src, tgt, state)
     dev = src.device
     n = src.shape[0] * int(K)
@@ -149,7 +168,8 @@
         out["cd"] = torch.empty((n, 8), dtype=_F32, device=dev)
     solve_iterate_out(src, tgt, state, K, steps_done, n_iters, angle_base, trans_mode, use_views, f64_params, k_full,
                       k_view, lr, betas[0], betas[1], eps, loss_scale, out["score"], out["loss"], out["R"], out["T"],
-                      out.get("grad"), out.get("cd"), nn_ws, -1 if ws_valid == "verify" else int(bool(ws_valid)), large=large)
+                      out.get("grad"), out.get("cd"), nn_ws, -1 if ws_valid == "verify" else int(bool(ws_valid)), large=large,
+                      chunk_iters=chunk_iters, sched_ws=sched_ws)
     return out
 
 
diff --git a/houv_amd/solver.py b/houv_amd/solver.py
--- a/houv_amd/solver.py
+++ b/houv_amd/solver.py
@@ -11,6 +11,22 @@
 ITERS_PER_LAUNCH = 50
 
 LAUNCH_LOG = None
+
+_STAGE_STATUS = []
+
+
+def check_stage_status(wait=False):
+    pending = []
+    for ws, ev in _STAGE_STATUS:
+        if wait:
+            ev.synchronize()
+        if not ev.query():
+            pending.append((ws, ev))
+        elif int(ws[1].item()) != 0:
+            _STAGE_STATUS.clear()
+            raise RuntimeError("houv_solve_stage: a workgroup's wait for the previous chunk of its hypothesis ran out of time "
+                               f"(status {int(ws[1].item())}); the stage's results are not valid")
+    _STAGE_STATUS[:] = pending
 
 LATTICE_AXES = np.array([(x, y, z) for x in (-1, 0, 1) for y in (-1, 0, 1) for z in (-1, 0, 1)
                          if (x, y, z) != (0, 0, 0)], dtype=np.float64)
@@ -336,6 +352,26 @@
         nn_ws = ops.solve_workspace(n, N, tgt.shape[1], dev)
     done, out = 0, None
     last_params = None
+    if not iters_per_launch and not want_last_params:
+        sched_ws = ops.solve_sched_workspace(n, dev)
+        if LAUNCH_LOG is not None:
+            ev0 = torch.cuda.Event(enable_timing=True)
+            ev1 = torch.cuda.Event(enable_timing=True)
+            ev0.record(torch.cuda.current_stream(dev))
+        out = ops.solve_iterate(src, tgt, state, K, steps_done=0, n_iters=n_iters, angle_base=angle_base,
+                                trans_mode=trans_mode, use_views=use_views, f64_params=f64_params, k_full=k_full,
+                                k_view=k_view, lr=lr, loss_scale=1.0 / n, want_grad=want_grad, want_cd=want_cd, nn_ws=nn_ws,
+                                ws_valid="verify" if pruned == "verify" else False, chunk_iters=step, sched_ws=sched_ws)
+        if LAUNCH_LOG is not None:
+            ev1.record(torch.cuda.current_stream(dev))
+            LAUNCH_LOG.append((ev0, ev1, n, n_iters, N, tgt.shape[1], bool(use_views), nn_ws is not None, True))
+        if src.is_cuda:
+            ev = torch.cuda.Event()
+            ev.record(torch.cuda.current_stream(dev))
+            if len(_STAGE_STATUS) >= 64:
+                check_stage_status(wait=True)
+            _STAGE_STATUS.append((sched_ws, ev))
+        return out, state
     while done < n_iters:
         it = min(step, n_iters - done)
         if want_last_params:
@@ -378,6 +414,7 @@
     score, R, T = stage_fn(src, tgt, 0)
     best, _ = score.topk(1, dim=1, largest=False, sorted=True)
     retry = torch.nonzero(best[:, 0] > RETRY_THRESHOLD).reshape(-1)
+    check_stage_status()
     if retry.numel() > 0:
         s_add, t_add = src[retry].contiguous(), tgt[retry].contiguous()
         for sub, whole in ((s_add, src), (t_add, tgt)):
@@ -410,6 +447,7 @@
             score[ge] = score_a[flag]
             T[ge] = T_a[flag]
             best[ge] = best_a[flag]
+        check_stage_status()
     _, k = score.topk(1, dim=1, largest=False, sorted=True)
     pick = k[:, 0]
     rows = torch.arange(B, device=score.device)
diff --git a/include/houv_hip.h b/include/houv_hip.h
--- a/include/houv_hip.h
+++ b/include/houv_hip.h
@@ -45,6 +45,24 @@
                               float* out_grad, float* out_cd,
                               int16_t* nn_ws, int ws_valid, int ws_stride, void* stream);
 
+int houv_solve_stage(const float* src, const float* tgt, int P, int N, int M, int K,
+                     double* state, int steps_done, int n_iters,
+                     int angle_base, int trans_mode, int use_views, int f64_params,
+                     int k_full, int k_view,
+                     double lr, double beta1, double beta2, double eps, float loss_scale,
+                     float* out_score, float* out_loss, float* out_R, float* out_T,
+                     float* out_grad, float* out_cd,
+                     int chunk_iters, int32_t* sched_ws, void* stream);
+int houv_solve_stage_pruned(const float* src, const float* tgt, int P, int N, int M, int K,
+                            double* state, int steps_done, int n_iters,
+                            int angle_base, int trans_mode, int use_views, int f64_params,
+                            int k_full, int k_view,
+                            double lr, double beta1, double beta2, double eps, float loss_scale,
+                            float* out_score, float* out_loss, float* out_R, float* out_T,
+                            float* out_grad, float* out_cd,
+                            int16_t* nn_ws, int ws_valid, int ws_stride,
+                            int chunk_iters, int32_t* sched_ws, void* stream);
+
 #define HOUV_LARGE_MAX_POINTS 16384
 int houv_solve_iterate_large(const float* src, const float* tgt, int P, int N, int M, int K,
                              double* state, int steps_done, int n_iters,
```

Result: faster. 230.2 pairs/s (median of 6 runs) (+7.1%).
